# ivannz/cplxmodule

Measured on AMD Instinct MI355X. Metric: Cplx-samples/sec fwd+bwd (CplxLinear-4096 + VD), higher is better.
Workload: dtype bf16; 1 GPU; CplxLinearVD 4096->4096, bf16 activations / fp32 master weights, batch 8192 per GPU, LRT fwd + KL + full bwd (BASELINE configs[1] + VD); global_batch=8192, parallelism=dp1, noise=in-kernel Philox4x32-7, launch=hipGraph replay, warmup_detail=5 eager steps (capture prerequisites) + 5 untimed replays

## Files before the change

cplxmodule_amd/_lib.py:

```python
import ctypes
import os
import threading
from ctypes import c_double, c_float, c_int, c_int64, c_uint64, c_void_p

import torch

_HERE = os.path.dirname(os.path.abspath(__file__))
LIB_PATH = os.environ.get("CPLXAMD_LIB") or os.path.join(_HERE, "libcplxamd.so")
ABI_VERSION = 25

F32, BF16, F16, F64 = 0, 1, 2, 3
KL_KINDS = {"real_vd": 0, "real_ard": 1, "cplx_vd": 2, "cplx_ard": 3, "cplx_vd_approx": 4,
            "cplx_vd_scalefree": 5, "cplx_vd_bogus": 6, "real_l0": 7, "real_l1": 8}

_P, _I, _L, _U, _F, _D = c_void_p, c_int, c_int64, c_uint64, c_float, c_double

SIGNATURES = {
    "cplxamd_abi_version": [],
    "cplxamd_vd_kl_ws_bytes": [],
    "cplxamd_vd_kl_fwd": [_P, _P, _P, _I, _P, _P, _P, _L, _P],
    "cplxamd_vd_kl_bwd": [_P, _P, _P, _I, _P, _P, _P, _P, _P, _L, _P],
    "cplxamd_vd_kl_fwd_bwd": [_P, _P, _P, _I, _F, _P, _P, _P, _P, _P, _L, _P],
    "cplxamd_vd_log_alpha": [_P, _P, _P, _P, _L, _P],
    "cplxamd_vd_log_alpha_bwd": [_P, _P, _P, _P, _P, _L, _P],
# ... 62 lines not shown
    "cplxamd_conv2d_cl2": [_P, _P, _P, _P, _P, _P, _P, _L] + [_I] * 11 + [_P, _L, _P],
    "cplxamd_chansum2": [_P, _P, _P, _P, _L, _I, _L, _I, _P, _P],
    "cplxamd_conv2d_cl2_lrt_dx": [_P] * 8 + [_L] + [_I] * 6 + [_P, _L, _P],
    "cplxamd_conv2d_cl2_mom_chunks": [_L] + [_I] * 10,
    "cplxamd_conv2d_cl2_mom": [_P, _P, _P, _P, _P, _P, _P, _L] + [_I] * 10 + [_P, _L, _P, _L, _P],
    "cplxamd_conv2d_cl_wgrad_ws_bytes": [_L, _I, _I, _I, _I],
    "cplxamd_conv2d_cl_wgrad": [_P, _P, _P, _P, _P, _P, _P, _L] + [_I] * 10 + [_P, _L, _P],
    "cplxamd_cgemm3m_ws_bytes": [_I, _I, _I],
    "cplxamd_abs2": [_P, _P, _P, _L, _I, _I, _P],
    "cplxamd_modulus": [_P, _P, _P, _L, _P],
    "cplxamd_exp": [_P, _P, _L, _I, _P],
    "cplxamd_cast": [_P, _P, _L, _I, _I, _P],
    "cplxamd_split3": [_P, _P, _L, _P, _L, _L, _L, _I, _I, _I, _P],
    "cplxamd_absmax_ws_bytes": [],
    "cplxamd_absmax_scale": [_P, _P, _L, _L, _I, _I, _P, _P, _P],
    "cplxamd_split2h": [_P, _P, _L, _P, _L, _L, _L, _I, _I, _I, _P, _P],
    "cplxamd_cgemm_sc_fl": [_P, _P, _L, _L, _P, _P, _L, _L, _P, _P, _P, _P, _P, _L, _I, _I, _I, _I, _I, _I, _P, _P, _P, _P, _L,
                            _I, _P],
    "cplxamd_rgemm_sc_fl": [_P, _L, _L, _P, _L, _L, _P, _P, _I, _P, _L, _I, _I, _I, _I, _I, _P, _P, _P, _P, _L, _I, _P],
    "cplxamd_transpose": [_P, _L, _P, _L, _I, _I, _I, _P],
    "cplxamd_colsum_ws_bytes": [_I],
    "cplxamd_colsum": [_P, _L, _P, _I, _I, _I, _P, _P],
    "cplxamd_colsum2": [_P, _P, _L, _P, _P, _I, _I, _I, _P, _P],
    "cplxamd_lrt_dx_accum": [_P, _P, _P, _P, _P, _L, _I, _I, _P],
    "cplxamd_conv2d_fwd": [_P, _P, _P, _P, _P, _P, _P, _P, _P, _I, _P],
    "cplxamd_conv2d_dgrad": [_P, _P, _P, _P, _P, _P, _P, _I, _P],
    "cplxamd_conv2d_wgrad_splits": [_P],
    "cplxamd_conv2d_wgrad_ws_bytes": [_P, _I],
    "cplxamd_conv2d_wgrad": [_P, _P, _P, _P, _P, _P, _P, _P, _I, _P, _L, _P],
    "cplxamd_conv2d_wgrad_bias": [_P, _P, _P, _P, _P, _P, _P, _P, _P, _P, _I, _P, _L, _P],
    "cplxamd_conv2d_out_shape": [_P, _P, _P],
    "cplxamd_conv2d_ktab_size": [_P, _I],
    "cplxamd_conv2d_ktab_fill": [_P, _I, _P],
    "cplxamd_conv2d_bf16_fwd": [_P, _P, _P, _P, _P, _P, _P, _P, _P, _P, _P],
    "cplxamd_conv2d_bf16_dgrad": [_P, _P, _P, _P, _P, _P, _P, _P, _P],
    "cplxamd_conv2d_bf16_wgrad_ws_bytes": [_P, _I],
    "cplxamd_conv2d_bf16_wgrad": [_P, _P, _P, _P, _P, _P, _P, _P, _P, _P, _L, _P],
    "cplxamd_chansum": [_P, _P, _L, _I, _L, _I, _P, _P],
    "cplxamd_bn_ws_bytes": [_I],
    "cplxamd_bn_fwd": [_P, _P, _P, _P, _L, _I, _L, _P, _P, _P, _P, _P, _I, _I, _F, _F, _P, _L, _P],
    "cplxamd_bn_fwd_ex": [_P, _P, _P, _P, _L, _I, _L, _P, _P, _P, _P, _P, _I, _I, _F, _F, _P, _P, _L, _P],
    "cplxamd_bn_bwd": [_P, _P, _P, _P, _P, _P, _L, _I, _L, _P, _P, _P, _P, _I, _I, _P, _L, _P],
    "cplxamd_bn_bwd_sums": [_P, _P, _P, _P, _P, _P, _L, _I, _L, _P, _P, _P, _P, _I, _I, _P, _P, _L, _P],
    "cplxamd_bn_rows_path": [_L, _I, _L],
    "cplxamd_gemm_set_persistent": [_I],
    "cplxamd_gemm_set_family": [_I],
    "cplxamd_cgemm_fl": [_P, _P, _L, _L, _P, _P, _L, _L, _P, _P, _P, _P, _P, _L, _I, _I, _I, _I, _I,
                         _I, _I, _P, _I, _P, _L, _I, _P],
    "cplxamd_rgemm_fl": [_P, _L, _L, _P, _L, _L, _P, _P, _I, _P, _L, _I, _I, _I, _I, _I, _I, _P, _P, _L, _I, _P],
    "cplxamd_cgemm_lrt_dx_fl": [_P, _P, _L, _L, _P, _P, _L, _L, _P, _P, _P, _L, _P, _P, _L, _I, _I, _I, _I, _I, _P],
    "cplxamd_rgemm_lrt_dx_fl": [_P, _L, _L, _P, _L, _L, _P, _P, _L, _P, _L, _I, _I, _I, _I, _I, _P],
    "cplxamd_gemm_plan": [_I] * 10,
    "cplxamd_conv2d_cl_fl": [_P, _P, _P, _P, _P, _P, _P, _L] + [_I] * 11 + [_P, _L, _I, _P],
    "cplxamd_conv2d_cl2_fl": [_P, _P, _P, _P, _P, _P, _P, _L] + [_I] * 11 + [_P, _L, _I, _P],
    "cplxamd_conv2d_cl2_lrt_dx_fl": [_P] * 8 + [_L] + [_I] * 6 + [_P, _L, _I, _P],
    "cplxamd_conv2d_cl2_mom_chunks_fl": [_L] + [_I] * 11,
    "cplxamd_conv2d_cl2_mom_fl": [_P, _P, _P, _P, _P, _P, _P, _L] + [_I] * 10 + [_P, _L, _P, _L, _I, _P],
    "cplxamd_conv2d_cl_wgrad_fl": [_P, _P, _P, _P, _P, _P, _P, _L] + [_I] * 10 + [_P, _L, _I, _P],
    "cplxamd_bn_bwd_sums_amax": [_P, _P, _P, _P, _P, _P, _L, _I, _L, _P, _P, _P, _P, _I, _I, _P, _P, _P, _L, _P],
    "cplxamd_absmax_scale_partials": [_P, _I, _P, _P],
    "cplxamd_bn_bwd_coef": [_P, _P, _P, _P, _L, _I, _L, _P, _P, _P, _P, _I, _I, _P, _P, _P, _L, _P],
    "cplxamd_conv2d_cl_wgrad_bn_fl": [_P] * 11 + [_L] + [_I] * 10 + [_P, _L, _I, _P],
    "cplxamd_gemm_f64": [_P, _P, _L, _L, _L, _P, _P, _L, _L, _L, _P, _P, _P, _P, _L, _L, _I, _I, _I, _I, _I, _P],
    "cplxamd_conv2d_f64": [_P, _P, _P, _P, _P, _P, _P, _P, _P, _I, _P],
    "cplxamd_expi_f64": [_P, _P, _L, _P],
    "cplxamd_conv2d_cl2h_fl": [_P, _P, _I, _P, _P, _P, _P, _P, _I, _P, _P, _L] + [_I] * 7 + [_P, _L, _I, _P],
    "cplxamd_conv2d_cl2h_wrap_fl": [_P, _P, _I, _I, _P, _P, _P, _P, _P, _I, _P, _P, _L] + [_I] * 7 + [_P, _L, _I, _P],
    "cplxamd_conv2d_clh_wgrad_ws_bytes": [_L, _I, _I, _I, _I],
    "cplxamd_conv2d_clh_wgrad": [_P, _P, _P, _P, _P, _P, _P, _L] + [_I] * 10 + [_P, _L, _P],
    "cplxamd_conv2d_clh_wgrad_fl": [_P, _P, _P, _P, _P, _P, _P, _L] + [_I] * 10 + [_P, _L, _I, _P],
    "cplxamd_conv2d_clh_wgrad_skip_fl": [_P, _P, _P, _P, _P, _P, _L] + [_I] * 12 + [_P, _L, _I, _P],
    "cplxamd_conv2d_clr_fl": [_P, _P, _P, _P, _L] + [_I] * 11 + [_P, _L, _I, _P],
    "cplxamd_conv2d_clr_wgrad_fl": [_P, _P, _P, _I, _P, _L] + [_I] * 10 + [_P, _L, _I, _P],
    "cplxamd_bn_moments": [_P, _P, _P, _P, _P, _L, _I, _L, _I, _P, _P, _L, _P],
    "cplxamd_bn_fwd_sync": [_P, _P, _P, _P, _L, _I, _L, _P, _P, _P, _P, _P, _I, _F, _F, _P, _P, _P, _L, _P],
    "cplxamd_bn_fwd_partials": [_P, _P, _P, _P, _L, _I, _L, _P, _P, _P, _P, _P, _I, _F, _F, _P, _P, _I, _P, _L, _P],
    "cplxamd_bn_bwd_sync": [_P, _P, _P, _P, _P, _P, _L, _I, _L, _P, _P, _P, _P, _I, _P, _P, _P, _P, _P, _L, _P],
    "cplxamd_cplx_fn_fwd": [_P, _P, _P, _P, _L, _I, _I, _P],
    "cplxamd_cplx_fn_bwd": [_P, _P, _P, _P, _P, _P, _L, _I, _I, _P],
    "cplxamd_welch_plan": [_L, _L, _L, _I, _P, _P],
    "cplxamd_welch_fwd": [_P, _P, _L, _L, _L, _L, _P, _L, _L, _I, _D, _P, _P, _L, _I, _P],
    "cplxamd_welch_bwd": [_P, _P, _L, _L, _L, _L, _P, _L, _L, _I, _D, _P, _P, _P, _L, _L, _P, _L, _I, _P],
    "cplxamd_ceinsum": [_P, _P, _P, _P, _P, _P, _P, _I, _I, _I, _I, _P],
}


class EinsumDesc(ctypes.Structure):
    _fields_ = [("nmodes", ctypes.c_int32 * 4), ("extent", (ctypes.c_int32 * 8) * 4), ("stride_a", (c_int64 * 8) * 4),
                ("stride_b", (c_int64 * 8) * 4), ("stride_c", (c_int64 * 8) * 4)]


CPLX_FN = {"exp": 0, "log": 1, "sin": 2, "cos": 3, "tan": 4, "sinh": 5, "cosh": 6, "tanh": 7}
_RESTYPES = {"cplxamd_absmax_ws_bytes": c_int64, "cplxamd_conv2d_cl2_mom_chunks": c_int64, "cplxamd_conv2d_cl2_mom_chunks_fl": c_int64, "cplxamd_vd_kl_ws_bytes": c_int64, "cplxamd_lrt_reparam_bwd_cols_ws_bytes": c_int64, "cplxamd_l0_gate_bwd_ws_bytes": c_int64, "cplxamd_bn_ws_bytes": c_int64,
             "cplxamd_conv2d_wgrad_ws_bytes": c_int64, "cplxamd_conv2d_bf16_wgrad_ws_bytes": c_int64, "cplxamd_colsum_ws_bytes": c_int64, "cplxamd_gemm_ws_bytes": c_int64,
             "cplxamd_cgemm3m_ws_bytes": c_int64,
             "cplxamd_conv2d_nhwc_wgrad_ws_bytes": c_int64,
             "cplxamd_conv2d_nhwc_wgrad_f32_ws_bytes": c_int64,
             "cplxamd_conv2d_cl_pack_bytes": c_int64, "cplxamd_conv2d_cl_ws_bytes": c_int64,
             "cplxamd_conv2d_cl_wgrad_ws_bytes": c_int64, "cplxamd_conv2d_clh_wgrad_ws_bytes": c_int64,

             "cplxamd_conv2d_clr_pack_bytes": c_int64,
             "cplxamd_conv2d_clr_ws_bytes": c_int64, "cplxamd_conv2d_clr_wgrad_ws_bytes": c_int64}

_lib = None

LAUNCH_DEFAULT, LAUNCH_SHARED, LAUNCH_EXCLUSIVE = 0, 1, 2


def LAUNCH_FAMILY(mask):
    return 0x100 | ((int(mask) & 0xff) << 16)


_policy = {}
_sharing = set()
_policy_lock = threading.Lock()


def _stream_key():
    if not torch.cuda.is_available():
        return (-1, 0)
    idx = torch.cuda.current_device()
    return (idx, _current_stream_handle(idx))


def launch_flags():
    if _policy:
        f = _policy.get(_stream_key())
        if f is not None:
            return f
    return LAUNCH_SHARED if _sharing else LAUNCH_DEFAULT


class launch_policy:

    def __init__(self, flags):
        self.flags = int(flags)

    def __enter__(self):
        self.key = _stream_key()
        with _policy_lock:
            self.prev = _policy.get(self.key)
            _policy[self.key] = self.flags
        return self

    def __exit__(self, *exc):
        with _policy_lock:
            if self.prev is None:
                _policy.pop(self.key, None)
            else:
                _policy[self.key] = self.prev
        return False


def shared_chip_enter(owner):
    with _policy_lock:
        _sharing.add(id(owner))


def shared_chip_leave(owner):
    with _policy_lock:
        _sharing.discard(id(owner))


class CplxAmdError(RuntimeError):
    pass


def load():
    global _lib
    if _lib is not None:
        return _lib
    if not os.path.exists(LIB_PATH):
        raise CplxAmdError(
            f"{LIB_PATH} not found: build it with `python -c 'import __graft_entry__ as g; "
            "g.build()'` (or cplxmodule_amd/csrc/build.sh).  cplxmodule_amd has no CPU or "
            "pure-torch fallback.")
# ... 98 lines not shown
```

cplxmodule_amd/csrc/common.h:

```cpp
#pragma once
#include <hip/hip_runtime.h>
#include <stdint.h>

#include "../../include/cplxamd.h"

#define CPLXAMD_CHECK_LAUNCH()                          \
  do {                                                  \
    hipError_t e__ = hipGetLastError();                 \
    if (e__ != hipSuccess) return (int)e__;             \
  } while (0)

#if defined(CPLXAMD_GEMM_F16) || defined(CPLXAMD_CONV_F16)
typedef _Float16 cplxamd_f16x8 __attribute__((ext_vector_type(8)));
#define CPLXAMD_MFMA16(a, b, c) \
  __builtin_amdgcn_mfma_f32_32x32x16_f16(__builtin_bit_cast(cplxamd_f16x8, a), __builtin_bit_cast(cplxamd_f16x8, b), c, 0, 0, 0)
#else
#define CPLXAMD_MFMA16(a, b, c) __builtin_amdgcn_mfma_f32_32x32x16_bf16(a, b, c, 0, 0, 0)
#endif

namespace cplxamd {

constexpr int kWave = 64;

#ifndef CPLXAMD_PHILOX_ROUNDS
// ... 51 lines not shown
                                             uint32_t lds_off_uniform) {
  const uint64_t a = (uint64_t)(uintptr_t)sbase_uniform;
  const uint64_t lo = (uint32_t)__builtin_amdgcn_readfirstlane((int)(uint32_t)a);
  const uint64_t hi = (uint32_t)__builtin_amdgcn_readfirstlane((int)(uint32_t)(a >> 32));
  const uint64_t sb = (hi << 32) | lo;
  const uint32_t m0v = (uint32_t)__builtin_amdgcn_readfirstlane((int)lds_off_uniform);
  asm volatile("s_mov_b32 m0, %0\n\ts_nop 0\n\tglobal_load_lds_dwordx4 %1, %2"
               :
               : "s"(m0v), "v"(voff), "s"(sb)
               : "memory");
}

struct f4 { float v[4]; };
struct f8 { f4 h[2]; };
__device__ __forceinline__ f4 ld4(const float* p) {
  float4 t = *reinterpret_cast<const float4*>(p);
  return f4{{t.x, t.y, t.z, t.w}};
}
__device__ __forceinline__ void st4(float* p, const f4& a) {
  *reinterpret_cast<float4*>(p) = make_float4(a.v[0], a.v[1], a.v[2], a.v[3]);
}
__device__ __forceinline__ f4 ld4(const bf16_t* p) {
  uint2 t = *reinterpret_cast<const uint2*>(p);
  return f4{{__uint_as_float(t.x << 16), __uint_as_float(t.x & 0xffff0000u),
             __uint_as_float(t.y << 16), __uint_as_float(t.y & 0xffff0000u)}};
}
__device__ __forceinline__ void st4(bf16_t* p, const f4& a) {
  uint2 t;
  t.x = pack_bf16(a.v[0], a.v[1]);
  t.y = pack_bf16(a.v[2], a.v[3]);
  *reinterpret_cast<uint2*>(p) = t;
}
__device__ __forceinline__ f8 ld8(const float* p) { return f8{{ld4(p), ld4(p + 4)}}; }
__device__ __forceinline__ void st8(float* p, const f8& a) { st4(p, a.h[0]); st4(p + 4, a.h[1]); }
__device__ __forceinline__ f8 ld8(const bf16_t* p) {
  const uint4 t = *reinterpret_cast<const uint4*>(p);
  const uint32_t w[4] = {t.x, t.y, t.z, t.w};
  f8 r;
#pragma unroll
  for (int e = 0; e < 4; ++e) {
    r.h[e >> 1].v[(e & 1) * 2] = __uint_as_float(w[e] << 16);
    r.h[e >> 1].v[(e & 1) * 2 + 1] = __uint_as_float(w[e] & 0xffff0000u);
  }
  return r;
}
__device__ __forceinline__ void st8(bf16_t* p, const f8& a) {
  uint32_t w[4];
#pragma unroll
  for (int e = 0; e < 4; ++e)
    w[e] = pack_bf16(a.h[e >> 1].v[(e & 1) * 2], a.h[e >> 1].v[(e & 1) * 2 + 1]);
  *reinterpret_cast<uint4*>(p) = uint4{w[0], w[1], w[2], w[3]};
}

__device__ __forceinline__ float rn_sqrt(float x) { return sqrtf(x); }

__device__ __forceinline__ float exact_logf(float x) {
  double d = (double)x;
  asm volatile("" : "+v"(d));
  return (float)log(d);
}

__device__ __forceinline__ double wave_sum(double v) {
#pragma unroll
  for (int o = 32; o > 0; o >>= 1) v += __shfl_xor(v, o, 64);
  return v;
}
__device__ __forceinline__ float wave_sum(float v) {
#pragma unroll
  for (int o = 32; o > 0; o >>= 1) v += __shfl_xor(v, o, 64);
  return v;
}

template <typename T, int NT>
__device__ __forceinline__ T block_sum(T v, T* smem) {
  v = wave_sum(v);
  const int lane = threadIdx.x & 63, wid = threadIdx.x >> 6;
  if (lane == 0) smem[wid] = v;
  __syncthreads();
  T r = T(0);
  if (threadIdx.x < NT / 64) r = smem[threadIdx.x];
  if (wid == 0) r = wave_sum(r);
  __syncthreads();
  return r;
}

__device__ __forceinline__ uint64_t uniform64(uint64_t v) {
  const uint32_t lo = (uint32_t)__builtin_amdgcn_readfirstlane((int)(uint32_t)v);
  const uint32_t hi = (uint32_t)__builtin_amdgcn_readfirstlane((int)(uint32_t)(v >> 32));
  return ((uint64_t)hi << 32) | lo;
}

struct u32x4 { uint32_t v[4]; };

__device__ __forceinline__ u32x4 philox4x32(uint64_t ctr_lo, uint64_t ctr_hi, uint64_t key) {
  uint32_t c0 = (uint32_t)ctr_lo, c1 = (uint32_t)(ctr_lo >> 32);
  uint32_t c2 = (uint32_t)ctr_hi, c3 = (uint32_t)(ctr_hi >> 32);
  uint32_t k0 = (uint32_t)key, k1 = (uint32_t)(key >> 32);
#pragma unroll
  for (int r = 0; r < kPhiloxRounds; ++r) {
    const uint64_t p0 = (uint64_t)0xD2511F53u * c0, p1 = (uint64_t)0xCD9E8D57u * c2;
    const uint32_t lo0 = (uint32_t)p0, hi0 = (uint32_t)(p0 >> 32);
    const uint32_t lo1 = (uint32_t)p1, hi1 = (uint32_t)(p1 >> 32);
    c0 = __builtin_amdgcn_bitop3_b32(hi1, c1, k0, 0x96);
    c1 = lo1;
    c2 = __builtin_amdgcn_bitop3_b32(hi0, c3, k1, 0x96);
    c3 = lo0;
    k0 += 0x9E3779B9u;
    k1 += 0xBB67AE85u;
  }
  return u32x4{{c0, c1, c2, c3}};
}

__device__ __forceinline__ float u01(uint32_t x) {
  return fmaf((float)(x >> 8), 5.9604644775390625e-08f, 2.98023223876953125e-08f);
}

inline int stream_grid(int64_t work_items, int block) {
  int64_t g = (work_items + block - 1) / block;
  if (g < 1) g = 1;
  if (g > 2048) g = 2048;
  return (int)g;
}

}
```

cplxmodule_amd/csrc/gemm_bf16_w4.hip:

```cpp
#include <stdlib.h>

#include <type_traits>

#include "gemm.h"

namespace cplxamd {
namespace w4 {

typedef __bf16 bf16x8 __attribute__((ext_vector_type(8)));
typedef short s16x4 __attribute__((ext_vector_type(4)));
typedef short s16x8 __attribute__((ext_vector_type(8)));
typedef float f32x16 __attribute__((ext_vector_type(16)));
typedef uint32_t u32x4 __attribute__((ext_vector_type(4)));

#ifndef W4_LDP
#define W4_LDP 0
#endif
#ifndef W4_WAIT1
#define W4_WAIT1 0
#endif
#ifndef W4_LDQ
#define W4_LDQ 0
#endif

// ... 450 lines not shown
        using NR = std::false_type;
        tile(I0{}, I0{}, t, NR{});
        tile(I1{}, I1{}, t + 1, NR{});
        tile(I2{}, I0{}, t + 2, NR{});
        tile(I0{}, I1{}, t + 3, NR{});
        tile(I1{}, I0{}, t + 4, NR{});
        tile(I2{}, I1{}, t + 5, NR{});
      }
    }
    for (; t + 6 <= nt; t += 6) {
      tile(I0{}, I0{}, t, RD{});
      tile(I1{}, I1{}, t + 1, RD{});
      tile(I2{}, I0{}, t + 2, RD{});
      tile(I0{}, I1{}, t + 3, RD{});
      tile(I1{}, I0{}, t + 4, RD{});
      tile(I2{}, I1{}, t + 5, RD{});
    }
    if (t < nt) {
      tile(I0{}, I0{}, t, RD{});
      tile(I1{}, I1{}, t + 1, RD{});
      t += 2;
      if (t < nt) {
        tile(I2{}, I0{}, t, RD{});
        tile(I0{}, I1{}, t + 1, RD{});
        if constexpr (PERSIST) rotate(I1{});
      } else {
        if constexpr (PERSIST) rotate(I2{});
      }
    }
  }

#ifdef CPLXAMD_GEMM_F16
  if constexpr (!PERSIST) {
    if (g.scale_a) {
      const float alpha = gemm_alpha(g);
#pragma unroll
      for (int i = 0; i < IB; ++i)
#pragma unroll
        for (int j = 0; j < JB; ++j) {
          acc_r[i][j] *= alpha;
          if (CPLX) acc_i[i][j] *= alpha;
        }
    }
  }
#endif

  void* out_r = g.c_r;
  void* out_i = g.c_i;
  if (g.splits > 1) {
    const int64_t slab = (int64_t)g.M * g.ldc;
    float* base = reinterpret_cast<float*>(g.ws) + (int64_t)split * NPL * slab;
    out_r = base; out_i = base + slab;
  }
  const float beta = gemm_beta(g);
  asm volatile("s_waitcnt lgkmcnt(0)" ::: "memory");
  if constexpr (!PERSIST) __builtin_amdgcn_s_barrier();
  auto tile_rsrc = [&](const void* plane, int64_t ld, int esize) __attribute__((always_inline)) {
    const char* base = (const char*)plane + ((int64_t)m0 * ld + n0) * esize;
    return __builtin_amdgcn_make_buffer_rsrc((void*)base, 0, 0x7ffffffe, 0x00020000);
  };
  auto ldb128 = [](__amdgpu_buffer_rsrc_t r, uint32_t vo, uint32_t so) __attribute__((always_inline)) -> u32x4 {
    return __builtin_amdgcn_raw_buffer_load_b128(r, vo, so, 0);
  };
  auto stb128 = [](u32x4 v, __amdgpu_buffer_rsrc_t r, uint32_t vo, uint32_t so) __attribute__((always_inline)) {
    __builtin_amdgcn_raw_buffer_store_b128(v, r, vo, so, 0);
  };
  if constexpr (sizeof(TOUT) == 2) {
    auto epi16 = [&](auto FUSE) __attribute__((always_inline)) {
      constexpr bool fuse = decltype(FUSE)::value;
      constexpr int PITCH = 144;
      const int tid_e = PERSIST ? (int)opaque((uint32_t)tid) : tid;
      const int lane = tid_e & 63, wid = tid_e >> 6;
      const int wm = (wid / C::WN) * (32 * IB), wn = (wid % C::WN) * (32 * JB);
      const int l31 = lane & 31, lk = lane >> 5;
      const uint32_t vo_c = (uint32_t)((((int64_t)(wm + (lane >> 3)) * g.ldc + wn + (lane & 7) * 8)) * 2);
      char* reg = smem + (PERSIST ? (CPLX ? sl[2] : (uint32_t)C::SMEM) : 0u) + wid * (64 * PITCH);
      const uint32_t vo_f = fuse ? (uint32_t)((((int64_t)(wm + (lane >> 3)) * g.fld + wn + (lane & 7) * 8)) * 2) : 0u;
      const uint32_t p8c = (uint32_t)__builtin_amdgcn_readfirstlane((int)(uint32_t)(8 * g.ldc * 2));
      const uint32_t p8f = (uint32_t)__builtin_amdgcn_readfirstlane((int)(uint32_t)(8 * g.fld * 2));
      const __amdgpu_buffer_rsrc_t rga = tile_rsrc(fuse ? g.fga : g.c_r, fuse ? g.fld : g.ldc, 2);
      const __amdgpu_buffer_rsrc_t rout0 = tile_rsrc(out_r, g.ldc, 2), rout1 = tile_rsrc(CPLX ? out_i : out_r, g.ldc, 2);
      const __amdgpu_buffer_rsrc_t rx0 = tile_rsrc(fuse ? g.fx_r : g.c_r, fuse ? g.fld : g.ldc, 2);
      const __amdgpu_buffer_rsrc_t rx1 = tile_rsrc(fuse ? (CPLX ? g.fx_i : g.fx_r) : g.c_r, fuse ? g.fld : g.ldc, 2);
      constexpr int NR = NPL * (JB / 2) * (IB / 2);
      u32x4 gv[2][fuse ? 8 : 1], xv[2][fuse ? 8 : 1];
      auto load_ops = [&](int r) __attribute__((always_inline)) {
        const int pl = r / ((JB / 2) * (IB / 2)), jh = (r / (IB / 2)) % (JB / 2), ih = r % (IB / 2);
#pragma unroll
        for (int pass = 0; pass < 8; ++pass) {
          const uint32_t so = (uint32_t)(ih * 8 + pass) * p8f + (uint32_t)(jh * 128);
          gv[r & 1][pass] = ldb128(rga, vo_f, so);
          xv[r & 1][pass] = ldb128(pl ? rx1 : rx0, vo_f, so);
        }
      };
      if constexpr (fuse) load_ops(0);
      if constexpr (PERSIST) W4_VMCNT(0);
#pragma unroll
      for (int r = 0; r < NR; ++r) {
        const int pl = r / ((JB / 2) * (IB / 2)), jh = (r / (IB / 2)) % (JB / 2), ih = r % (IB / 2);
        const __amdgpu_buffer_rsrc_t rout = pl ? rout1 : rout0;
        if constexpr (fuse && !W4_EPI_PIPE) { if (r > 0) load_ops(r); }
#pragma unroll
        for (int ii = 0; ii < 2; ++ii)
#pragma unroll
          for (int jj = 0; jj < 2; ++jj)
#pragma unroll
            for (int q = 0; q < 4; ++q) {
              const int cl = jj * 32 + 8 * q + 4 * lk;
              f4 v;
#pragma unroll
              for (int e = 0; e < 4; ++e) {
                const float a = pl ? acc_i[CPLX ? ih * 2 + ii : 0][jh * 2 + jj][4 * q + e] : acc_r[ih * 2 + ii][jh * 2 + jj][4 * q + e];
                v.v[e] = a;
              }
              st4(reinterpret_cast<bf16_t*>(reg + (ii * 32 + l31) * PITCH + cl * 2), v);
              if constexpr (PERSIST) W4_SB();
            }
        asm volatile("s_waitcnt lgkmcnt(0)" ::: "memory");
        if constexpr (fuse && W4_EPI_PIPE) {
          if (r + 1 < NR) { W4_SB(); load_ops(r + 1); W4_SB(); }
        }
#pragma unroll
        for (int pass = 0; pass < 8; ++pass) {
          const int rl = pass * 8 + (lane >> 3), c8 = (lane & 7) * 8;
          const u32x4 v = *reinterpret_cast<const u32x4*>(reg + rl * PITCH + c8 * 2);
          const uint32_t so = (uint32_t)(ih * 8 + pass) * p8c + (uint32_t)(jh * 128);
          if constexpr (fuse) {
            u32x4 ow;
#pragma unroll
            for (int e = 0; e < 4; ++e) {
              const float d0 = __uint_as_float(v[e] << 16), d1 = __uint_as_float(v[e] & 0xffff0000u);
              const float x0 = __uint_as_float(xv[r & 1][pass][e] << 16), x1 = __uint_as_float(xv[r & 1][pass][e] & 0xffff0000u);
              const float g0 = __uint_as_float(gv[r & 1][pass][e] << 16), g1 = __uint_as_float(gv[r & 1][pass][e] & 0xffff0000u);
              ow[e] = pack_bf16(fmaf(2.0f * x0, g0, d0), fmaf(2.0f * x1, g1, d1));
            }
            stb128(ow, rout, vo_c, so);
          } else {
            stb128(v, rout, vo_c, so);
          }
        }
        asm volatile("s_waitcnt lgkmcnt(0)" ::: "memory");
        if constexpr (PERSIST) W4_VMCNT(16);
        W4_SB();
      }
    };
    if constexpr (PERSIST) epi16(std::false_type{});
    else { if (g.fga) epi16(std::true_type{}); else epi16(std::false_type{}); }
  } else {
    auto epi32 = [&](auto HM, auto HACC) __attribute__((always_inline)) {
      constexpr bool hm = decltype(HM)::value, hacc = decltype(HACC)::value;
      constexpr int PITCH = 272;
      char* reg = smem + wid * (32 * PITCH);
      const uint32_t vo = (uint32_t)((((int64_t)(wm + (lane >> 4)) * g.ldc + wn + (lane & 15) * 4)) * 4);
      const uint32_t p4 = (uint32_t)__builtin_amdgcn_readfirstlane((int)(uint32_t)(4 * g.ldc * 4));
      const __amdgpu_buffer_rsrc_t rm = tile_rsrc(hm ? (const void*)g.emul : g.c_r, g.ldc, 4);
      const __amdgpu_buffer_rsrc_t rout0 = tile_rsrc(out_r, g.ldc, 4), rout1 = tile_rsrc(CPLX ? out_i : out_r, g.ldc, 4);
      constexpr int NR = NPL * (JB / 2) * IB;
      u32x4 mv[2][hm ? 8 : 1], pv[2][hacc ? 8 : 1];
      auto load_ops = [&](int r) __attribute__((always_inline)) {
        const int pl = r / ((JB / 2) * IB), jh = (r / IB) % (JB / 2), i = r % IB;
#pragma unroll
        for (int pass = 0; pass < 8; ++pass) {
          const uint32_t so = (uint32_t)(i * 8 + pass) * p4 + (uint32_t)(jh * 256);
          if constexpr (hm) mv[r & 1][pass] = ldb128(rm, vo, so);
          if constexpr (hacc) pv[r & 1][pass] = ldb128(pl ? rout1 : rout0, vo, so);
        }
      };
      if constexpr (hm || hacc) load_ops(0);
#pragma unroll
      for (int r = 0; r < NR; ++r) {
        const int pl = r / ((JB / 2) * IB), jh = (r / IB) % (JB / 2), i = r % IB;
        const __amdgpu_buffer_rsrc_t rout = pl ? rout1 : rout0;
        if constexpr ((hm || hacc) && !W4_EPI_PIPE) { if (r > 0) load_ops(r); }
#pragma unroll
        for (int jj = 0; jj < 2; ++jj)
#pragma unroll
          for (int q = 0; q < 4; ++q) {
            const int cl = jj * 32 + 8 * q + 4 * lk;
            f4 v;
#pragma unroll
            for (int e = 0; e < 4; ++e)
              v.v[e] = pl ? acc_i[CPLX ? i : 0][jh * 2 + jj][4 * q + e] : acc_r[i][jh * 2 + jj][4 * q + e];
            st4(reinterpret_cast<float*>(reg + l31 * PITCH + cl * 4), v);
          }
        asm volatile("s_waitcnt lgkmcnt(0)" ::: "memory");
        if constexpr ((hm || hacc) && W4_EPI_PIPE) {
          if (r + 1 < NR) { W4_SB(); load_ops(r + 1); W4_SB(); }
        }
#pragma unroll
        for (int pass = 0; pass < 8; ++pass) {
          const int rl = pass * 4 + (lane >> 4), c4 = (lane & 15) * 4;
          f4 v = ld4(reinterpret_cast<const float*>(reg + rl * PITCH + c4 * 4));
          const uint32_t so = (uint32_t)(i * 8 + pass) * p4 + (uint32_t)(jh * 256);
          if constexpr (hm) {
#pragma unroll
            for (int e = 0; e < 4; ++e) {
              v.v[e] *= gemm_emul(g, __uint_as_float(mv[r & 1][pass][e]));
              asm volatile("" : "+v"(v.v[e]));
            }
          }
          if constexpr (hacc) {
#pragma unroll
            for (int e = 0; e < 4; ++e) v.v[e] += beta * __uint_as_float(pv[r & 1][pass][e]);
          }
          const u32x4 w = {__float_as_uint(v.v[0]), __float_as_uint(v.v[1]), __float_as_uint(v.v[2]), __float_as_uint(v.v[3])};
          stb128(w, rout, vo, so);
        }
        asm volatile("s_waitcnt lgkmcnt(0)" ::: "memory");
        W4_SB();
      }
    };
    if (g.emul) { if (g.accumulate) epi32(std::true_type{}, std::true_type{}); else epi32(std::true_type{}, std::false_type{}); }
    else { if (g.accumulate) epi32(std::false_type{}, std::true_type{}); else epi32(std::false_type{}, std::false_type{}); }
  }
  if constexpr (!PERSIST) {
    break;
// ... 144 lines not shown
```

cplxmodule_amd/csrc/kl.hip:

```cpp
#include "common.h"

#pragma clang fp contract(off)

namespace cplxamd {

constexpr int kKlThreads = 256;
constexpr int kKlMaxBlocks = 2048;
#ifndef KL_UNROLL
#define KL_UNROLL 1
#endif
#ifndef KL_NT
#define KL_NT 3
#endif

constexpr float kEulerGamma = 0.57721566490153286f;
constexpr float kK1 = 0.63576f, kK2 = 1.87320f, kK3 = 1.48695f;

template <bool CPLX, bool EXACT = true>
__device__ __forceinline__ float weight_abs(float wr, float wi) {
  if (CPLX) return EXACT ? rn_sqrt(fmaf(wi, wi, wr * wr)) : __builtin_amdgcn_sqrtf(fmaf(wi, wi, wr * wr));
  return fabsf(wr);
}

template <bool CPLX, bool EXACT>
// ... 96 lines not shown
template <int KIND>
__device__ __forceinline__ float one_param_value(float p, float& slope) {
  if (KIND == CPLXAMD_KL_REAL_L0) {
    const float s = sigmoid_f(kL0Shift - p);
    slope = -(s * (1.0f - s));
    return s;
  }
  slope = p > 0.0f ? 1.0f : (p < 0.0f ? -1.0f : 0.0f);
  return fabsf(p);
}

template <bool CPLX>
__device__ __forceinline__ void weight_grad(float fp, float wr, float wi, float theta,
                                            float& gwr, float& gwi) {
  if (theta > 0.0f) {
    if (CPLX) {
      const float c = 2.0f * fp * __builtin_amdgcn_rcpf(theta * (theta + 1e-12f));
      gwr = c * wr;
      gwi = c * wi;
    } else {
      gwr = (wr < 0.0f ? -2.0f : 2.0f) * fp / (theta + 1e-12f);
      gwi = 0.0f;
    }
  } else {
    gwr = 0.0f;
    gwi = 0.0f;
  }
}

typedef float f2 __attribute__((ext_vector_type(2)));
__device__ __forceinline__ f2 fma2(f2 a, f2 b, f2 c) { return __builtin_elementwise_fma(a, b, c); }
__device__ __forceinline__ f2 sp2(float v) { return f2{v, v}; }
__device__ __forceinline__ f2 sel2(bool c0, bool c1, f2 a, f2 b) { return f2{c0 ? a.x : b.x, c1 ? a.y : b.y}; }

__device__ __forceinline__ float exp_neg(float ls) {
  const float yh = -ls * 1.44269504089f;
  const float yl = fmaf(-ls, 1.44269504089f, -yh);
  const float e = __builtin_amdgcn_exp2f(yh);
  return fmaf(e, yl * 0.69314718056f, e);
}

__device__ __forceinline__ void cplx_vd_pair(f2 x, f2& val, f2& slope) {
  f2 s = sp2(3.0619244e-7f);
  s = fma2(s, x, sp2(-3.1001984e-6f));
  s = fma2(s, x, sp2(2.8344671e-5f));
  s = fma2(s, x, sp2(-2.3148148e-4f));
  s = fma2(s, x, sp2(1.6666667e-3f));
  s = fma2(s, x, sp2(-1.0416667e-2f));
  s = fma2(s, x, sp2(5.5555556e-2f));
  s = fma2(s, x, sp2(-0.25f));
  s = fma2(s, x, sp2(1.0f));
  const f2 small = s * x;
  const f2 num = fma2(fma2(fma2(x + sp2(8.5733287401f), x, sp2(18.0590169730f)), x, sp2(8.6347608925f)), x, sp2(0.2677737343f));
  const f2 den = fma2(fma2(fma2(x + sp2(9.5733223454f), x, sp2(25.6329561486f)), x, sp2(21.0996530827f)), x, sp2(3.9584969228f));
  const f2 xd = x * den;
  const f2 nx = x * sp2(-1.44269504089f);
  const f2 e = f2{__builtin_amdgcn_exp2f(nx.x), __builtin_amdgcn_exp2f(nx.y)};
  const f2 rc = f2{__builtin_amdgcn_rcpf(xd.x), __builtin_amdgcn_rcpf(xd.y)};
  const f2 lg = f2{__builtin_amdgcn_logf(x.x), __builtin_amdgcn_logf(x.y)} * sp2(0.69314718056f);
  f2 e1 = e * num * rc;
  e1 = sel2(x.x < 104.0f, x.y < 104.0f, e1, sp2(0.0f));
  const f2 large = sp2(kEulerGamma) + lg + e1;
  val = sel2(x.x <= 1.0f, x.y <= 1.0f, small, large);
  const f2 ss = fma2(fma2(x, sp2(1.6666667e-1f), sp2(-0.5f)), x, sp2(1.0f)) * x;
  slope = sel2(x.x < 0.015625f, x.y < 0.015625f, ss, sp2(1.0f) - e);
}

struct KlArgs {
  const float* wr;
  const float* wi;
  const float* ls2;
  const float* g_elem;
  const float* g_scalar;
  float gscale;
  float* out_elem;
  double* partial;
  float* g_ls2;
  float* g_wr;
  float* g_wi;
  int64_t n;
  bf16_t* wr_b = nullptr;
  bf16_t* wi_b = nullptr;
  bf16_t* s_b = nullptr;
};

__device__ __forceinline__ void st4g(float* p, const f4& v) {
#if KL_NT & 1
  typedef float f4v __attribute__((ext_vector_type(4)));
  __builtin_nontemporal_store(f4v{v.v[0], v.v[1], v.v[2], v.v[3]}, reinterpret_cast<f4v*>(p));
#else
  st4(p, v);
#endif
}
__device__ __forceinline__ f4 ld4g(const float* p) {
#if KL_NT & 2
  typedef float f4v __attribute__((ext_vector_type(4)));
  const f4v t = __builtin_nontemporal_load(reinterpret_cast<const f4v*>(p));
  return f4{{t.x, t.y, t.z, t.w}};
#else
  return ld4(p);
#endif
}

template <int KIND, bool VALUE, bool GRAD>
__global__ __launch_bounds__(kKlThreads) void kl_kernel(KlArgs a) {
  constexpr bool CPLX = KIND >= CPLXAMD_KL_CPLX_VD && KIND <= CPLXAMD_KL_CPLX_VD_BOGUS;
  constexpr float kLs = kl_ls2_term<KIND>();
  __shared__ double red[kKlThreads / 64];
  const int64_t n4 = a.n >> 2;
  const int64_t stride = (int64_t)gridDim.x * kKlThreads;
  float gs = a.gscale;
  if (GRAD && a.g_scalar) gs *= *a.g_scalar;
  double acc = 0.0;

  auto body = [&](int64_t i, const f4& wr, const f4& ls, const f4& wi, const f4& ge) __attribute__((always_inline)) {
    f4 val, d_ls, d_wr, d_wi;
    float part = 0.0f;
    bool done = false;
    if constexpr (KIND == CPLXAMD_KL_CPLX_VD) {
      float q[4];
      bool tiny = false;
#pragma unroll
      for (int j = 0; j < 4; ++j) {
        q[j] = fmaf(wi.v[j], wi.v[j], wr.v[j] * wr.v[j]);
        tiny |= !(q[j] >= 1e-8f);
      }
#pragma unroll
      for (int h = 0; h < 2; ++h) {
        const f2 x = f2{q[2 * h] * exp_neg(ls.v[2 * h]), q[2 * h + 1] * exp_neg(ls.v[2 * h + 1])};
        f2 v, sl;
        cplx_vd_pair(x, v, sl);
        if (VALUE) { val.v[2 * h] = v.x; val.v[2 * h + 1] = v.y; }
        if (GRAD) {
          const f2 fp = sl * f2{ge.v[2 * h], ge.v[2 * h + 1]} * sp2(gs);
          const f2 c = (fp + fp) * f2{__builtin_amdgcn_rcpf(q[2 * h]), __builtin_amdgcn_rcpf(q[2 * h + 1])};
          d_ls.v[2 * h] = -fp.x; d_ls.v[2 * h + 1] = -fp.y;
          d_wr.v[2 * h] = c.x * wr.v[2 * h]; d_wr.v[2 * h + 1] = c.y * wr.v[2 * h + 1];
          d_wi.v[2 * h] = c.x * wi.v[2 * h]; d_wi.v[2 * h + 1] = c.y * wi.v[2 * h + 1];
        }
      }
      done = !tiny;
      if (VALUE && done) part = (val.v[0] + val.v[1]) + (val.v[2] + val.v[3]);
    }
    if constexpr (kl_one_param<KIND>()) {
#pragma unroll
      for (int j = 0; j < 4; ++j) {
        float sl;
        const float v = one_param_value<KIND>(KIND == CPLXAMD_KL_REAL_L0 ? ls.v[j] : wr.v[j], sl);
        if (VALUE) { val.v[j] = v; part += v; }
        if (GRAD) {
          const float g = sl * ge.v[j] * gs;
          d_ls.v[j] = KIND == CPLXAMD_KL_REAL_L0 ? g : 0.0f;
          d_wr.v[j] = KIND == CPLXAMD_KL_REAL_L1 ? g : 0.0f;
          d_wi.v[j] = 0.0f;
        }
      }
      done = true;
    }
    if (!done) {
      part = 0.0f;
#pragma unroll
      for (int j = 0; j < 4; ++j) {
        float theta;
        const float t = -log_alpha_of<CPLX, false>(ls.v[j], wr.v[j], wi.v[j], theta);
        if (VALUE) {
          val.v[j] = kl_value<KIND>(t) + kLs * ls.v[j];
// ... 4 lines not shown
          d_ls.v[j] = kLs * ge.v[j] * gs - fp;
          weight_grad<CPLX>(fp, wr.v[j], wi.v[j], theta, d_wr.v[j], d_wi.v[j]);
        }
      }
    }
    if (VALUE) {
      acc += (double)part;
      if (a.out_elem) st4(a.out_elem + 4 * i, val);
    }
    if (GRAD) {
      if (a.g_ls2) st4g(a.g_ls2 + 4 * i, d_ls);
      if (a.g_wr) st4g(a.g_wr + 4 * i, d_wr);
      if (CPLX && a.g_wi) st4g(a.g_wi + 4 * i, d_wi);
    }
    if (a.wr_b) st4(a.wr_b + 4 * i, wr);
    if (CPLX && a.wi_b) st4(a.wi_b + 4 * i, wi);
    if (a.s_b) {
      f4 e;
#pragma unroll
      for (int j = 0; j < 4; ++j) e.v[j] = expf(ls.v[j]);
      st4(a.s_b + 4 * i, e);
    }
  };
  for (int64_t i0 = (int64_t)blockIdx.x * kKlThreads + threadIdx.x; i0 < n4; i0 += KL_UNROLL * stride) {
    f4 wr[KL_UNROLL], ls[KL_UNROLL], wi[KL_UNROLL], ge[KL_UNROLL];
#pragma unroll
    for (int u = 0; u < KL_UNROLL; ++u) {
      const int64_t i = i0 + u * stride;
      wi[u] = f4{{0.f, 0.f, 0.f, 0.f}};
      ge[u] = f4{{1.f, 1.f, 1.f, 1.f}};
      if (i < n4) {
        wr[u] = ld4g(a.wr + 4 * i);
        ls[u] = ld4g(a.ls2 + 4 * i);
        if (CPLX) wi[u] = ld4g(a.wi + 4 * i);
        if (GRAD && a.g_elem) ge[u] = ld4(a.g_elem + 4 * i);
      }
    }
#pragma unroll
    for (int u = 0; u < KL_UNROLL; ++u) {
      const int64_t i = i0 + u * stride;
      if (i < n4) body(i, wr[u], ls[u], wi[u], ge[u]);
    }
  }
  if (blockIdx.x == 0) {
    const int64_t i = (n4 << 2) + threadIdx.x;
    if (i < a.n) {
      const float wr = a.wr[i], ls = a.ls2[i];
      const float wi = CPLX ? a.wi[i] : 0.0f;
      if constexpr (kl_one_param<KIND>()) {
        float sl;
        const float v = one_param_value<KIND>(KIND == CPLXAMD_KL_REAL_L0 ? ls : wr, sl);
        if (VALUE) {
          acc += (double)v;
          if (a.out_elem) a.out_elem[i] = v;
        }
        if (GRAD) {
          const float g = sl * (a.g_elem ? a.g_elem[i] : 1.0f) * gs;
          if (a.g_ls2) a.g_ls2[i] = KIND == CPLXAMD_KL_REAL_L0 ? g : 0.0f;
          if (a.g_wr) a.g_wr[i] = KIND == CPLXAMD_KL_REAL_L1 ? g : 0.0f;
        }
      } else {
      float theta;
      const float t = -log_alpha_of<CPLX, false>(ls, wr, wi, theta);
      if (VALUE) {
        const float v = kl_value<KIND>(t) + kLs * ls;
        acc += (double)v;
        if (a.out_elem) a.out_elem[i] = v;
      }
      if (GRAD) {
        const float ge = a.g_elem ? a.g_elem[i] : 1.0f;
        const float fp = kl_slope<KIND>(t) * ge * gs;
        float gwr, gwi;
        weight_grad<CPLX>(fp, wr, wi, theta, gwr, gwi);
        if (a.g_ls2) a.g_ls2[i] = kLs * ge * gs - fp;
        if (a.g_wr) a.g_wr[i] = gwr;
        if (CPLX && a.g_wi) a.g_wi[i] = gwi;
      }
      }
    }
  }
  if (VALUE && a.partial) {
    const double s = block_sum<double, kKlThreads>(acc, red);
    if (threadIdx.x == 0) a.partial[blockIdx.x] = s;
  }
}

__global__ __launch_bounds__(kKlThreads) void kl_final_kernel(const double* partial, int m,
                                                              float* out) {
  __shared__ double red[kKlThreads / 64];
  double acc = 0.0;
  for (int i = threadIdx.x; i < m; i += kKlThreads) acc += partial[i];
  const double s = block_sum<double, kKlThreads>(acc, red);
  if (threadIdx.x == 0) *out = (float)s;
}

template <bool VALUE, bool GRAD>
static int launch_kl(int kind, const KlArgs& a, int grid, hipStream_t st) {
  switch (kind) {
    case CPLXAMD_KL_REAL_VD:
      kl_kernel<CPLXAMD_KL_REAL_VD, VALUE, GRAD><<<grid, kKlThreads, 0, st>>>(a);
      break;
    case CPLXAMD_KL_REAL_ARD:
      kl_kernel<CPLXAMD_KL_REAL_ARD, VALUE, GRAD><<<grid, kKlThreads, 0, st>>>(a);
      break;
    case CPLXAMD_KL_CPLX_VD:
      kl_kernel<CPLXAMD_KL_CPLX_VD, VALUE, GRAD><<<grid, kKlThreads, 0, st>>>(a);
      break;
    case CPLXAMD_KL_CPLX_ARD:
      kl_kernel<CPLXAMD_KL_CPLX_ARD, VALUE, GRAD><<<grid, kKlThreads, 0, st>>>(a);
      break;
    case CPLXAMD_KL_CPLX_VD_APPROX:
      kl_kernel<CPLXAMD_KL_CPLX_VD_APPROX, VALUE, GRAD><<<grid, kKlThreads, 0, st>>>(a);
      break;
    case CPLXAMD_KL_CPLX_VD_SCALEFREE:
      kl_kernel<CPLXAMD_KL_CPLX_VD_SCALEFREE, VALUE, GRAD><<<grid, kKlThreads, 0, st>>>(a);
      break;
    case CPLXAMD_KL_CPLX_VD_BOGUS:
      kl_kernel<CPLXAMD_KL_CPLX_VD_BOGUS, VALUE, GRAD><<<grid, kKlThreads, 0, st>>>(a);
      break;
    case CPLXAMD_KL_REAL_L0:
      kl_kernel<CPLXAMD_KL_REAL_L0, VALUE, GRAD><<<grid, kKlThreads, 0, st>>>(a);
      break;
    case CPLXAMD_KL_REAL_L1:
      kl_kernel<CPLXAMD_KL_REAL_L1, VALUE, GRAD><<<grid, kKlThreads, 0, st>>>(a);
      break;
    default:
      return CPLXAMD_EINVAL;
  }
  CPLXAMD_CHECK_LAUNCH();
  return 0;
}

__global__ __launch_bounds__(kKlThreads) void prep_kernel(const float* wr, const float* wi, const float* ls2,
                                                          bf16_t* wr_b, bf16_t* wi_b, bf16_t* s_b, int64_t n) {
  const int64_t n4 = n >> 2, stride = (int64_t)gridDim.x * kKlThreads;
  for (int64_t i = (int64_t)blockIdx.x * kKlThreads + threadIdx.x; i < n4; i += stride) {
    if (wr_b) st4(wr_b + 4 * i, ld4(wr + 4 * i));
    if (wi_b) st4(wi_b + 4 * i, ld4(wi + 4 * i));
    if (s_b) {
      f4 e = ld4(ls2 + 4 * i);
#pragma unroll
      for (int j = 0; j < 4; ++j) e.v[j] = expf(e.v[j]);
      st4(s_b + 4 * i, e);
    }
  }
}

static bool kl_args_ok(const float* wr, const float* wi, const float* ls2, int kind, int64_t n) {
  if (!wr || !ls2 || n < 0 || kind < 0 || kind > CPLXAMD_KL_REAL_L1) return false;
  const bool cplx = kind >= CPLXAMD_KL_CPLX_VD && kind <= CPLXAMD_KL_CPLX_VD_BOGUS;
  return cplx ? wi != nullptr : true;
}

template <bool CPLX, bool MASK>
__global__ __launch_bounds__(kKlThreads) void log_alpha_kernel(const float* wr, const float* wi,
                                                               const float* ls2, float thr,
                                                               float* out, double* partial,
                                                               int64_t n) {
  __shared__ double red[kKlThreads / 64];
  const int64_t n4 = n >> 2;
  const int64_t stride = (int64_t)gridDim.x * kKlThreads;
  double cnt = 0.0;
  for (int64_t i = (int64_t)blockIdx.x * kKlThreads + threadIdx.x; i < n4; i += stride) {
    const f4 a = ld4(wr + 4 * i), l = ld4(ls2 + 4 * i);
    f4 b = {{0.f, 0.f, 0.f, 0.f}};
    if (CPLX) b = ld4(wi + 4 * i);
    f4 o;
    float c = 0.0f;
#pragma unroll
    for (int j = 0; j < 4; ++j) {
      float theta;
      const float la = log_alpha_of<CPLX, true>(l.v[j], a.v[j], b.v[j], theta);
      o.v[j] = MASK ? (la <= thr ? 1.0f : 0.0f) : la;
      c += MASK ? o.v[j] : 0.0f;
    }
    st4(out + 4 * i, o);
    cnt += (double)c;
  }
  if (blockIdx.x == 0) {
    const int64_t i = (n4 << 2) + threadIdx.x;
    if (i < n) {
      float theta;
      const float la = log_alpha_of<CPLX, true>(ls2[i], wr[i], CPLX ? wi[i] : 0.0f, theta);
      const float o = MASK ? (la <= thr ? 1.0f : 0.0f) : la;
      out[i] = o;
      if (MASK) cnt += (double)o;
    }
  }
  if (MASK && partial) {
    const double s = block_sum<double, kKlThreads>(cnt, red);
    if (threadIdx.x == 0) partial[blockIdx.x] = s;
  }
}

template <bool CPLX>
__global__ __launch_bounds__(kKlThreads) void log_alpha_bwd_kernel(const float* g, const float* wr,
                                                                   const float* wi, float* g_wr, float* g_wi,
                                                                   int64_t n) {
  const int64_t stride = (int64_t)gridDim.x * kKlThreads;
  for (int64_t i = (int64_t)blockIdx.x * kKlThreads + threadIdx.x; i < n; i += stride) {
    const float a = wr[i], b = CPLX ? wi[i] : 0.0f;
    const float theta = weight_abs<CPLX, true>(a, b);
    float ga, gb;
    weight_grad<CPLX>(-g[i], a, b, theta, ga, gb);
    g_wr[i] = ga;
    if (CPLX) g_wi[i] = gb;
  }
}

__global__ __launch_bounds__(kKlThreads) void count_final_kernel(const double* partial, int m,
                                                                 int64_t* out) {
  __shared__ double red[kKlThreads / 64];
  double acc = 0.0;
  for (int i = threadIdx.x; i < m; i += kKlThreads) acc += partial[i];
  const double s = block_sum<double, kKlThreads>(acc, red);
  if (threadIdx.x == 0) *out = (int64_t)(s + 0.5);
}

__device__ __forceinline__ float expi_f(float xf) {
  const double x = (double)xf;
  if (xf == 0.0f) return -INFINITY;
  if (xf < 0.0f) {
    const double y = -x;
    if (y <= 1.0) {
      double s = 0.0, term = 1.0;
      for (int k = 1; k <= 20; ++k) {
        term *= -y / k;
        s += term / k;
      }
      return (float)(0.57721566490153286 + log(y) + s);
    }
    if (y > 745.0) return -0.0f;
    double b = y + 1.0, c = 1e300, d = 1.0 / b, h = d;
    for (int i = 1; i <= 60; ++i) {
      const double an = -(double)i * i;
      b += 2.0;
      d = 1.0 / (an * d + b);
      c = b + an / c;
      const double del = c * d;
      h *= del;
      if (fabs(del - 1.0) < 1e-15) break;
    }
    return (float)(-h * exp(-y));
  }
  if (x <= 40.0) {
    double s = 0.0, term = 1.0;
    for (int k = 1; k <= 200; ++k) {
      term *= x / k;
      const double add = term / k;
      s += add;
      if (add < s * 1e-17) break;
    }
    return (float)(0.57721566490153286 + log(x) + s);
  }
  double s = 1.0, term = 1.0;
  for (int k = 1; k <= 40; ++k) {
    const double nt = term * k / x;
    if (nt > term) break;
    term = nt;
    s += term;
  }
  return (float)(exp(x) / x * s);
}

__global__ __launch_bounds__(kKlThreads) void expi_fwd_kernel(const float* x, float* y, int64_t n) {
  const int64_t stride = (int64_t)gridDim.x * kKlThreads;
  for (int64_t i = (int64_t)blockIdx.x * kKlThreads + threadIdx.x; i < n; i += stride)
    y[i] = expi_f(x[i]);
}
__global__ __launch_bounds__(kKlThreads) void expi_bwd_kernel(const float* g, const float* x,
                                                              float* gx, int64_t n) {
  const int64_t stride = (int64_t)gridDim.x * kKlThreads;
  for (int64_t i = (int64_t)blockIdx.x * kKlThreads + threadIdx.x; i < n; i += stride)
    gx[i] = g[i] * expf(x[i]) / x[i];
}

}

using namespace cplxamd;

extern "C" {

int cplxamd_abi_version(void) { return CPLXAMD_ABI_VERSION; }

int64_t cplxamd_vd_kl_ws_bytes(void) { return (int64_t)kKlMaxBlocks * sizeof(double); }

int cplxamd_vd_kl_fwd(const float* wr, const float* wi, const float* log_sigma2, int kind,
                      float* out_elem, float* out_sum, void* ws, int64_t n, void* stream) {
  if (!kl_args_ok(wr, wi, log_sigma2, kind, n) || (out_sum && !ws)) return CPLXAMD_EINVAL;
  hipStream_t st = (hipStream_t)stream;
  const int grid = stream_grid(n >> 2, kKlThreads);
  KlArgs a{wr, wi, log_sigma2, nullptr, nullptr, 1.0f, out_elem,
           out_sum ? (double*)ws : nullptr, nullptr, nullptr, nullptr, n};
  int rc = launch_kl<true, false>(kind, a, grid, st);
  if (rc) return rc;
  if (out_sum) {
    kl_final_kernel<<<1, kKlThreads, 0, st>>>((const double*)ws, grid, out_sum);
    CPLXAMD_CHECK_LAUNCH();
  }
  return 0;
}

int cplxamd_vd_kl_bwd(const float* wr, const float* wi, const float* log_sigma2, int kind,
                      const float* g_elem, const float* g_scalar, float* g_log_sigma2,
                      float* g_wr, float* g_wi, int64_t n, void* stream) {
  if (!kl_args_ok(wr, wi, log_sigma2, kind, n)) return CPLXAMD_EINVAL;
  const int grid = stream_grid(n >> 2, kKlThreads);
  KlArgs a{wr, wi, log_sigma2, g_elem, g_scalar, 1.0f, nullptr, nullptr,
           g_log_sigma2, g_wr, g_wi, n};
  return launch_kl<false, true>(kind, a, grid, (hipStream_t)stream);
}

int cplxamd_vd_kl_fwd_bwd(const float* wr, const float* wi, const float* log_sigma2, int kind,
                          float gscale, float* out_sum, float* g_log_sigma2, float* g_wr,
                          float* g_wi, void* ws, int64_t n, void* stream) {
  if (!kl_args_ok(wr, wi, log_sigma2, kind, n) || !out_sum || !ws) return CPLXAMD_EINVAL;
  hipStream_t st = (hipStream_t)stream;
  const int grid = stream_grid(n >> 2, kKlThreads);
  KlArgs a{wr, wi, log_sigma2, nullptr, nullptr, gscale, nullptr, (double*)ws,
           g_log_sigma2, g_wr, g_wi, n};
  int rc = launch_kl<true, true>(kind, a, grid, st);
  if (rc) return rc;
  kl_final_kernel<<<1, kKlThreads, 0, st>>>((const double*)ws, grid, out_sum);
  CPLXAMD_CHECK_LAUNCH();
  return 0;
}

int cplxamd_vd_prep_kl(const float* wr, const float* wi, const float* log_sigma2, int kind, int with_kl,
                       void* wr_bf16, void* wi_bf16, void* s_bf16, float* out_sum, float* g_log_sigma2,
                       float* g_wr, float* g_wi, void* ws, int64_t n, void* stream) {
  if (n < 0 || (n & 3)) return CPLXAMD_ESHAPE;
  if ((wr_bf16 && !wr) || (wi_bf16 && !wi) || (s_bf16 && !log_sigma2)) return CPLXAMD_EINVAL;
  hipStream_t st = (hipStream_t)stream;
  const int grid = stream_grid(n >> 2, kKlThreads);
  if (!with_kl) {
    prep_kernel<<<grid, kKlThreads, 0, st>>>(wr, wi, log_sigma2, (bf16_t*)wr_bf16, (bf16_t*)wi_bf16,
                                             (bf16_t*)s_bf16, n);
    CPLXAMD_CHECK_LAUNCH();
    return 0;
  }
  if (!kl_args_ok(wr, wi, log_sigma2, kind, n) || !out_sum || !ws) return CPLXAMD_EINVAL;
  KlArgs a{wr, wi, log_sigma2, nullptr, nullptr, 1.0f, nullptr, (double*)ws,
           g_log_sigma2, g_wr, g_wi, n};
  a.wr_b = (bf16_t*)wr_bf16; a.wi_b = (bf16_t*)wi_bf16; a.s_b = (bf16_t*)s_bf16;
  int rc = launch_kl<true, true>(kind, a, grid, st);
  if (rc) return rc;
  kl_final_kernel<<<1, kKlThreads, 0, st>>>((const double*)ws, grid, out_sum);
  CPLXAMD_CHECK_LAUNCH();
  return 0;
}

int cplxamd_vd_log_alpha(const float* wr, const float* wi, const float* log_sigma2, float* out,
                         int64_t n, void* stream) {
  if (!wr || !log_sigma2 || !out || n < 0) return CPLXAMD_EINVAL;
  hipStream_t st = (hipStream_t)stream;
  const int grid = stream_grid(n >> 2, kKlThreads);
  if (wi)
    log_alpha_kernel<true, false><<<grid, kKlThreads, 0, st>>>(wr, wi, log_sigma2, 0.f, out,
                                                               nullptr, n);
  else
    log_alpha_kernel<false, false><<<grid, kKlThreads, 0, st>>>(wr, wi, log_sigma2, 0.f, out,
                                                                nullptr, n);
  CPLXAMD_CHECK_LAUNCH();
  return 0;
}

int cplxamd_vd_log_alpha_bwd(const float* g, const float* wr, const float* wi, float* g_wr, float* g_wi,
                             int64_t n, void* stream) {
  if (!g || !wr || !g_wr || n < 0 || ((wi == nullptr) != (g_wi == nullptr))) return CPLXAMD_EINVAL;
  hipStream_t st = (hipStream_t)stream;
  const int grid = stream_grid(n, kKlThreads);
  if (wi) log_alpha_bwd_kernel<true><<<grid, kKlThreads, 0, st>>>(g, wr, wi, g_wr, g_wi, n);
  else log_alpha_bwd_kernel<false><<<grid, kKlThreads, 0, st>>>(g, wr, wi, g_wr, g_wi, n);
  CPLXAMD_CHECK_LAUNCH();
  return 0;
}

int cplxamd_vd_mask(const float* wr, const float* wi, const float* log_sigma2, float threshold,
                    float* mask, int64_t* count, void* ws, int64_t n, void* stream) {
  if (!wr || !log_sigma2 || !mask || n < 0 || (count && !ws)) return CPLXAMD_EINVAL;
  hipStream_t st = (hipStream_t)stream;
  const int grid = stream_grid(n >> 2, kKlThreads);
  double* partial = count ? (double*)ws : nullptr;
  if (wi)
    log_alpha_kernel<true, true><<<grid, kKlThreads, 0, st>>>(wr, wi, log_sigma2, threshold,
                                                              mask, partial, n);
  else
    log_alpha_kernel<false, true><<<grid, kKlThreads, 0, st>>>(wr, wi, log_sigma2, threshold,
                                                               mask, partial, n);
  CPLXAMD_CHECK_LAUNCH();
  if (count) {
    count_final_kernel<<<1, kKlThreads, 0, st>>>(partial, grid, count);
    CPLXAMD_CHECK_LAUNCH();
  }
  return 0;
}

int cplxamd_expi_fwd(const float* x, float* y, int64_t n, void* stream) {
  if (!x || !y || n < 0) return CPLXAMD_EINVAL;
  expi_fwd_kernel<<<stream_grid(n, kKlThreads), kKlThreads, 0, (hipStream_t)stream>>>(x, y, n);
  CPLXAMD_CHECK_LAUNCH();
  return 0;
}

int cplxamd_expi_bwd(const float* g, const float* x, float* gx, int64_t n, void* stream) {
  if (!g || !x || !gx || n < 0) return CPLXAMD_EINVAL;
  expi_bwd_kernel<<<stream_grid(n, kKlThreads), kKlThreads, 0, (hipStream_t)stream>>>(g, x, gx, n);
  CPLXAMD_CHECK_LAUNCH();
  return 0;
}

}
```

cplxmodule_amd/csrc/reparam.hip:

```cpp
#include "common.h"

#pragma clang fp contract(off)

namespace cplxamd {

constexpr int kRpThreads = 256;

__device__ __forceinline__ void box_muller(uint32_t a, uint32_t b, float scale, float& z0,
                                           float& z1) {
  const float r = __builtin_amdgcn_sqrtf((-1.3862943611198906f * scale * scale) * __builtin_amdgcn_logf(u01(a)));
  const float ang = u01(b);
  z0 = r * __builtin_amdgcn_cosf(ang);
  z1 = r * __builtin_amdgcn_sinf(ang);
}

__device__ __forceinline__ f4 philox_normals(uint64_t group, uint64_t seed, uint64_t offset,
                                             float scale) {
  const u32x4 x = philox4x32(group, offset, seed);
  f4 z;
  box_muller(x.v[0], x.v[1], scale, z.v[0], z.v[1]);
  box_muller(x.v[2], x.v[3], scale, z.v[2], z.v[3]);
  return z;
}

constexpr float kRsqrt2 = 0.70710678118654752f;

template <bool CPLX>
__device__ __forceinline__ void noise_vec(int64_t i4, uint64_t seed, uint64_t offset, f4& er,
                                          f4& ei) {
  if (CPLX) {
    const f4 a = philox_normals(2 * (uint64_t)i4, seed, offset, kRsqrt2);
    const f4 b = philox_normals(2 * (uint64_t)i4 + 1, seed, offset, kRsqrt2);
    er = f4{{a.v[0], a.v[2], b.v[0], b.v[2]}};
    ei = f4{{a.v[1], a.v[3], b.v[1], b.v[3]}};
  } else {
    er = philox_normals((uint64_t)i4, seed, offset, 1.0f);
  }
}

template <bool CPLX>
__device__ __forceinline__ void noise_one(int64_t e, uint64_t seed, uint64_t offset, float& er,
                                          float& ei) {
  if (CPLX) {
    const f4 a = philox_normals((uint64_t)e >> 1, seed, offset, kRsqrt2);
    er = (e & 1) ? a.v[2] : a.v[0];
    ei = (e & 1) ? a.v[3] : a.v[1];
  } else {
    const f4 a = philox_normals((uint64_t)e >> 2, seed, offset, 1.0f);
    er = a.v[e & 3];
    ei = 0.0f;
  }
}

__device__ __forceinline__ float lrt_std(float s2) { return rn_sqrt(fmaxf(s2, 1e-8f)); }

template <typename T> __device__ __forceinline__ float lrt_std_t(float s2) {
  if (sizeof(T) == 2) return __builtin_amdgcn_sqrtf(fmaxf(s2, 1e-8f));
  return lrt_std(s2);
}

template <typename T, typename TS, bool CPLX, bool PHILOX>
__global__ __launch_bounds__(kRpThreads) void reparam_fwd_kernel(
    const T* mu_r, const T* mu_i, const TS* s2, const T* eps_r, const T* eps_i, uint64_t seed,
    uint64_t offset, const uint64_t* state, T* y_r, T* y_i, int64_t n) {
  if (PHILOX && state) { seed = uniform64(state[0]); offset = uniform64(state[1]); }
  const int64_t n8 = n >> 3;
  const int64_t stride = (int64_t)gridDim.x * kRpThreads;
  for (int64_t i = (int64_t)blockIdx.x * kRpThreads + threadIdx.x; i < n8; i += stride) {
    const f8 s = ld8(s2 + 8 * i);
    const f8 mr = ld8(mu_r + 8 * i);
    f8 mi, er, ei, yr, yi;
    if (CPLX) mi = ld8(mu_i + 8 * i);
    if (!PHILOX) {
      er = ld8(eps_r + 8 * i);
      if (CPLX) ei = ld8(eps_i + 8 * i);
    }
#pragma unroll
    for (int h = 0; h < 2; ++h) {
      if (PHILOX) noise_vec<CPLX>(2 * i + h, seed, offset, er.h[h], ei.h[h]);
#pragma unroll
      for (int j = 0; j < 4; ++j) {
        const float sd = lrt_std_t<T>(s.h[h].v[j]);
        yr.h[h].v[j] = mr.h[h].v[j] + er.h[h].v[j] * sd;
        if (CPLX) yi.h[h].v[j] = mi.h[h].v[j] + ei.h[h].v[j] * sd;
      }
    }
    st8(y_r + 8 * i, yr);
    if (CPLX) st8(y_i + 8 * i, yi);
  }
  if (blockIdx.x == 0) {
    const int64_t e = (n8 << 3) + threadIdx.x;
    if (e < n) {
      float er, ei = 0.0f;
      if (PHILOX) {
        noise_one<CPLX>(e, seed, offset, er, ei);
      } else {
        er = io<T>::ld(eps_r + e);
        if (CPLX) ei = io<T>::ld(eps_i + e);
      }
      const float sd = lrt_std_t<T>(io<TS>::ld(s2 + e));
      io<T>::st(y_r + e, io<T>::ld(mu_r + e) + er * sd);
      if (CPLX) io<T>::st(y_i + e, io<T>::ld(mu_i + e) + ei * sd);
    }
  }
}

__device__ __forceinline__ float lrt_gs2(float gs, float s2) {
  return s2 >= 1e-8f ? (gs * 0.5f) / lrt_std(s2) : 0.0f;
}
template <typename T> __device__ __forceinline__ float lrt_gs2_t(float gs, float s2) {
  if (sizeof(T) == 2) return s2 >= 1e-8f ? (gs * 0.5f) * __builtin_amdgcn_rsqf(s2) : 0.0f;
  return lrt_gs2(gs, s2);
}

template <typename T, typename TG, typename TS, bool CPLX, bool PHILOX>
__global__ __launch_bounds__(kRpThreads) void reparam_bwd_kernel(
    const T* g_r, const T* g_i, const TS* s2, const T* eps_r, const T* eps_i, uint64_t seed,
    uint64_t offset, const uint64_t* state, TG* g_s2, int64_t n) {
  if (PHILOX && state) { seed = uniform64(state[0]); offset = uniform64(state[1]); }
  const int64_t n8 = n >> 3;
  const int64_t stride = (int64_t)gridDim.x * kRpThreads;
  for (int64_t i = (int64_t)blockIdx.x * kRpThreads + threadIdx.x; i < n8; i += stride) {
    const f8 s = ld8(s2 + 8 * i);
    const f8 gr = ld8(g_r + 8 * i);
    f8 gi, er, ei, o;
    if (CPLX) gi = ld8(g_i + 8 * i);
    if (!PHILOX) {
      er = ld8(eps_r + 8 * i);
      if (CPLX) ei = ld8(eps_i + 8 * i);
    }
#pragma unroll
    for (int h = 0; h < 2; ++h) {
      if (PHILOX) noise_vec<CPLX>(2 * i + h, seed, offset, er.h[h], ei.h[h]);
#pragma unroll
      for (int j = 0; j < 4; ++j) {
        float gs = gr.h[h].v[j] * er.h[h].v[j];
        if (CPLX) gs = gs + gi.h[h].v[j] * ei.h[h].v[j];
        o.h[h].v[j] = lrt_gs2_t<T>(gs, s.h[h].v[j]);
      }
    }
    st8(g_s2 + 8 * i, o);
  }
  if (blockIdx.x == 0) {
    const int64_t e = (n8 << 3) + threadIdx.x;
    if (e < n) {
      float er, ei = 0.0f;
      if (PHILOX) {
        noise_one<CPLX>(e, seed, offset, er, ei);
      } else {
        er = io<T>::ld(eps_r + e);
        if (CPLX) ei = io<T>::ld(eps_i + e);
      }
      float gs = io<T>::ld(g_r + e) * er;
      if (CPLX) gs = gs + io<T>::ld(g_i + e) * ei;
      io<TG>::st(g_s2 + e, lrt_gs2_t<T>(gs, io<TS>::ld(s2 + e)));
    }
  }
}

template <typename T, typename TG, typename TS, bool CPLX, bool PHILOX>
__global__ __launch_bounds__(kRpThreads) void reparam_bwd_cols_kernel(
    const T* g_r, const T* g_i, const TS* s2, const T* eps_r, const T* eps_i, uint64_t seed,
    uint64_t offset, const uint64_t* state, TG* g_s2, int64_t rows, int cols, int64_t rows_per_chunk,
    float* partial) {
  __shared__ float red[kRpThreads * 16];
  if (PHILOX && state) { seed = uniform64(state[0]); offset = uniform64(state[1]); }
  const int CG = cols >> 3;
  const int TX = CG < kRpThreads ? CG : kRpThreads, TY = kRpThreads / TX;
  const int tx = (int)threadIdx.x % TX, ty = (int)threadIdx.x / TX;
  const int col = (int)blockIdx.x * (kRpThreads * 8) + tx * 8;
  const int64_t r0 = (int64_t)blockIdx.y * rows_per_chunk;
  const int64_t r1 = r0 + rows_per_chunk < rows ? r0 + rows_per_chunk : rows;
  constexpr int NP = CPLX ? 2 : 1;
  float acc[NP][8];
#pragma unroll
  for (int p = 0; p < NP; ++p)
#pragma unroll
    for (int c = 0; c < 8; ++c) acc[p][c] = 0.0f;
  for (int64_t r = r0 + ty; r < r1; r += TY) {
    const int64_t i = (r * cols + col) >> 3;
    const f8 s = ld8(s2 + 8 * i);
    const f8 gr = ld8(g_r + 8 * i);
    f8 gi, er, ei, o;
    if (CPLX) gi = ld8(g_i + 8 * i);
    if (!PHILOX) {
      er = ld8(eps_r + 8 * i);
      if (CPLX) ei = ld8(eps_i + 8 * i);
    }
#pragma unroll
    for (int h = 0; h < 2; ++h) {
      if (PHILOX) noise_vec<CPLX>(2 * i + h, seed, offset, er.h[h], ei.h[h]);
#pragma unroll
      for (int j = 0; j < 4; ++j) {
        float gs = gr.h[h].v[j] * er.h[h].v[j];
        if (CPLX) gs = gs + gi.h[h].v[j] * ei.h[h].v[j];
        o.h[h].v[j] = lrt_gs2_t<T>(gs, s.h[h].v[j]);
        acc[0][4 * h + j] += gr.h[h].v[j];
        if (CPLX) acc[NP - 1][4 * h + j] += gi.h[h].v[j];
      }
    }
    st8(g_s2 + 8 * i, o);
  }
  float* dst = partial + (int64_t)blockIdx.y * NP * cols;
  if (TY == 1) {
#pragma unroll
    for (int p = 0; p < NP; ++p) {
      st4(dst + (int64_t)p * cols + col, f4{{acc[p][0], acc[p][1], acc[p][2], acc[p][3]}});
      st4(dst + (int64_t)p * cols + col + 4, f4{{acc[p][4], acc[p][5], acc[p][6], acc[p][7]}});
    }
    return;
  }
#pragma unroll
  for (int p = 0; p < NP; ++p)
#pragma unroll
    for (int c = 0; c < 8; ++c) red[((ty * NP + p) * TX + tx) * 8 + c] = acc[p][c];
  __syncthreads();
  for (int f = (int)threadIdx.x; f < NP * cols; f += kRpThreads) {
    const int p = f / cols, c = f % cols;
    float t = 0.0f;
    for (int l = 0; l < TY; ++l) t += red[((l * NP + p) * TX) * 8 + c];
    dst[(int64_t)p * cols + c] = t;
  }
}

__global__ __launch_bounds__(1024) void reparam_cols_final(const float* partial, int chunks, int cols, int planes,
                                                           float* out_r, float* out_i) {
  __shared__ float red[64][17];
  const int tx = threadIdx.x & 15, ty = threadIdx.x >> 4;
  const int c = blockIdx.x * 16 + tx, n = planes * cols;
  float acc = 0.f;
  if (c < n)
    for (int j = ty; j < chunks; j += 64) acc += partial[(int64_t)j * n + c];
  red[ty][tx] = acc;
  __syncthreads();
  if (ty == 0 && c < n) {
    float t = 0.f;
#pragma unroll 8
    for (int l = 0; l < 64; ++l) t += red[l][tx];
    if (c < cols) out_r[c] = t;
    else out_i[c - cols] = t;
  }
}

struct ColsPlan { int strips, chunks; int64_t rows_per_chunk; };
static bool cols_plan(int64_t rows, int cols, ColsPlan& p) {
  if (rows <= 0 || cols < 8 || cols % 8) return false;
  const int cg = cols / 8;
  if (cg < kRpThreads ? (kRpThreads % cg != 0) : (cols % (kRpThreads * 8) != 0)) return false;
  if (rows * (int64_t)cols >= ((int64_t)1 << 40)) return false;
  p.strips = cg < kRpThreads ? 1 : cols / (kRpThreads * 8);
  const int ty = cg < kRpThreads ? kRpThreads / cg : 1;
  int64_t chunks = rows / (16 * (int64_t)ty);
  const int64_t cap = 2048 / p.strips > 0 ? 2048 / p.strips : 1;
  if (chunks > cap) chunks = cap;
  if (chunks < 1) chunks = 1;
  int64_t rpc = (rows + chunks - 1) / chunks;
  rpc = (rpc + ty - 1) / ty * ty;
  p.rows_per_chunk = rpc;
  p.chunks = (int)((rows + rpc - 1) / rpc);
  return p.chunks <= 65535;
}

template <typename T, typename TG, typename TS>
static int launch_bwd_cols(const void* g_r, const void* g_i, const void* s2, const void* eps_r,
                           const void* eps_i, uint64_t seed, uint64_t offset, const uint64_t* state,
                           void* g_s2, int64_t rows, int cols, const ColsPlan& p, float* partial, hipStream_t st) {
  const dim3 grid((unsigned)p.strips, (unsigned)p.chunks);
  const bool cplx = g_i != nullptr, philox = eps_r == nullptr;
#define RP_BWDC(C, P)                                                                          \
  reparam_bwd_cols_kernel<T, TG, TS, C, P><<<grid, kRpThreads, 0, st>>>(                       \
      (const T*)g_r, (const T*)g_i, (const TS*)s2, (const T*)eps_r, (const T*)eps_i, seed, offset, \
      state, (TG*)g_s2, rows, cols, p.rows_per_chunk, partial)
  if (cplx && philox) RP_BWDC(true, true);
  else if (cplx) RP_BWDC(true, false);
  else if (philox) RP_BWDC(false, true);
  else RP_BWDC(false, false);
#undef RP_BWDC
  CPLXAMD_CHECK_LAUNCH();
  return 0;
}

template <bool CPLX>
__global__ __launch_bounds__(kRpThreads) void philox_normal_kernel(float* er, float* ei,
                                                                   uint64_t seed, uint64_t offset,
                                                                   int64_t n) {
  const int64_t stride = (int64_t)gridDim.x * kRpThreads;
  for (int64_t e = (int64_t)blockIdx.x * kRpThreads + threadIdx.x; e < n; e += stride) {
    float a, b;
    noise_one<CPLX>(e, seed, offset, a, b);
    er[e] = a;
    if (CPLX) ei[e] = b;
  }
}

template <typename T, typename TS>
static int launch_fwd(const void* mu_r, const void* mu_i, const void* s2, const void* eps_r,
                      const void* eps_i, uint64_t seed, uint64_t offset, const uint64_t* state,
                      void* y_r, void* y_i, int64_t n, hipStream_t st) {
  const int grid = stream_grid(n >> 3, kRpThreads);
  const bool cplx = mu_i != nullptr, philox = eps_r == nullptr;
#define RP_FWD(C, P)                                                                       \
  reparam_fwd_kernel<T, TS, C, P><<<grid, kRpThreads, 0, st>>>(                            \
      (const T*)mu_r, (const T*)mu_i, (const TS*)s2, (const T*)eps_r, (const T*)eps_i, seed, offset,  \
      state, (T*)y_r, (T*)y_i, n)
  if (cplx && philox) RP_FWD(true, true);
  else if (cplx) RP_FWD(true, false);
  else if (philox) RP_FWD(false, true);
  else RP_FWD(false, false);
#undef RP_FWD
  CPLXAMD_CHECK_LAUNCH();
  return 0;
}

template <typename T, typename TG, typename TS>
static int launch_bwd(const void* g_r, const void* g_i, const void* s2, const void* eps_r,
                      const void* eps_i, uint64_t seed, uint64_t offset, const uint64_t* state,
                      void* g_s2, int64_t n, hipStream_t st) {
  const int grid = stream_grid(n >> 3, kRpThreads);
  const bool cplx = g_i != nullptr, philox = eps_r == nullptr;
#define RP_BWD(C, P)                                                                      \
  reparam_bwd_kernel<T, TG, TS, C, P><<<grid, kRpThreads, 0, st>>>(                       \
      (const T*)g_r, (const T*)g_i, (const TS*)s2, (const T*)eps_r, (const T*)eps_i, seed, offset,   \
      state, (TG*)g_s2, n)
  if (cplx && philox) RP_BWD(true, true);
  else if (cplx) RP_BWD(true, false);
  else if (philox) RP_BWD(false, true);
  else RP_BWD(false, false);
#undef RP_BWD
  CPLXAMD_CHECK_LAUNCH();
  return 0;
}

__global__ void philox_advance_kernel(uint64_t* state, uint64_t* used) {
  if (threadIdx.x == 0 && blockIdx.x == 0) {
    used[0] = state[0];
    used[1] = state[1];
    state[1] = state[1] + 1;
  }
}

}

using namespace cplxamd;

static bool al16(const void* p) { return (reinterpret_cast<uintptr_t>(p) & 15) == 0; }

extern "C" {

int cplxamd_lrt_reparam_fwd_ex(const void* mu_r, const void* mu_i, const void* s2,
                               const void* eps_r, const void* eps_i, uint64_t seed,
                               uint64_t offset, const uint64_t* state, void* y_r, void* y_i,
                               int64_t n, int dtype, int s2_dtype, void* stream) {
  if (!mu_r || !s2 || !y_r || n < 0) return CPLXAMD_EINVAL;
  if (!al16(mu_r) || !al16(mu_i) || !al16(s2) || !al16(eps_r) || !al16(eps_i) || !al16(y_r) || !al16(y_i))
    return CPLXAMD_EALIGN;
  if ((mu_i == nullptr) != (y_i == nullptr)) return CPLXAMD_EINVAL;
  if (eps_r && mu_i && !eps_i) return CPLXAMD_EINVAL;
  hipStream_t st = (hipStream_t)stream;
  if (dtype == CPLXAMD_F32 && s2_dtype == CPLXAMD_F32)
    return launch_fwd<float, float>(mu_r, mu_i, s2, eps_r, eps_i, seed, offset, state, y_r, y_i, n, st);
  if (dtype == CPLXAMD_BF16 && s2_dtype == CPLXAMD_F32)
    return launch_fwd<bf16_t, float>(mu_r, mu_i, s2, eps_r, eps_i, seed, offset, state, y_r, y_i, n, st);
  if (dtype == CPLXAMD_BF16 && s2_dtype == CPLXAMD_BF16)
    return launch_fwd<bf16_t, bf16_t>(mu_r, mu_i, s2, eps_r, eps_i, seed, offset, state, y_r, y_i, n, st);
  return CPLXAMD_EINVAL;
}

int cplxamd_lrt_reparam_fwd(const void* mu_r, const void* mu_i, const float* s2,
                            const void* eps_r, const void* eps_i, uint64_t seed,
                            uint64_t offset, const uint64_t* state, void* y_r, void* y_i,
                            int64_t n, int dtype, void* stream) {
  return cplxamd_lrt_reparam_fwd_ex(mu_r, mu_i, s2, eps_r, eps_i, seed, offset, state, y_r, y_i, n, dtype,
                                    CPLXAMD_F32, stream);
}

int cplxamd_lrt_reparam_bwd_ex(const void* g_r, const void* g_i, const void* s2,
                               const void* eps_r, const void* eps_i, uint64_t seed,
                               uint64_t offset, const uint64_t* state, void* g_s2, int64_t n,
                               int dtype, int gs2_dtype, int s2_dtype, void* stream) {
  if (!g_r || !s2 || !g_s2 || n < 0) return CPLXAMD_EINVAL;
  if (eps_r && g_i && !eps_i) return CPLXAMD_EINVAL;
  if (!al16(g_r) || !al16(g_i) || !al16(s2) || !al16(eps_r) || !al16(eps_i) || !al16(g_s2))
    return CPLXAMD_EALIGN;
  hipStream_t st = (hipStream_t)stream;
  if (dtype == CPLXAMD_F32 && gs2_dtype == CPLXAMD_F32 && s2_dtype == CPLXAMD_F32)
    return launch_bwd<float, float, float>(g_r, g_i, s2, eps_r, eps_i, seed, offset, state, g_s2, n, st);
  if (dtype == CPLXAMD_BF16 && gs2_dtype == CPLXAMD_F32 && s2_dtype == CPLXAMD_F32)
    return launch_bwd<bf16_t, float, float>(g_r, g_i, s2, eps_r, eps_i, seed, offset, state, g_s2, n, st);
  if (dtype == CPLXAMD_BF16 && gs2_dtype == CPLXAMD_BF16 && s2_dtype == CPLXAMD_F32)
    return launch_bwd<bf16_t, bf16_t, float>(g_r, g_i, s2, eps_r, eps_i, seed, offset, state, g_s2, n, st);
  if (dtype == CPLXAMD_BF16 && gs2_dtype == CPLXAMD_BF16 && s2_dtype == CPLXAMD_BF16)
    return launch_bwd<bf16_t, bf16_t, bf16_t>(g_r, g_i, s2, eps_r, eps_i, seed, offset, state, g_s2, n, st);
  if (dtype == CPLXAMD_BF16 && gs2_dtype == CPLXAMD_F32 && s2_dtype == CPLXAMD_BF16)
    return launch_bwd<bf16_t, float, bf16_t>(g_r, g_i, s2, eps_r, eps_i, seed, offset, state, g_s2, n, st);
  return CPLXAMD_EINVAL;
}

int cplxamd_lrt_reparam_bwd(const void* g_r, const void* g_i, const float* s2,
                            const void* eps_r, const void* eps_i, uint64_t seed,
                            uint64_t offset, const uint64_t* state, void* g_s2, int64_t n,
                            int dtype, int gs2_dtype, void* stream) {
  return cplxamd_lrt_reparam_bwd_ex(g_r, g_i, s2, eps_r, eps_i, seed, offset, state, g_s2, n, dtype, gs2_dtype,
                                    CPLXAMD_F32, stream);
}

int64_t cplxamd_lrt_reparam_bwd_cols_ws_bytes(int64_t rows, int cols) {
  ColsPlan p;
  if (!cols_plan(rows, cols, p)) return 0;
  return (int64_t)p.chunks * 2 * cols * (int64_t)sizeof(float);
}

int cplxamd_lrt_reparam_bwd_cols(const void* g_r, const void* g_i, const void* s2,
                                 const void* eps_r, const void* eps_i, uint64_t seed,
                                 uint64_t offset, const uint64_t* state, void* g_s2, int64_t rows,
                                 int cols, int dtype, int gs2_dtype, int s2_dtype, float* sum_r,
                                 float* sum_i, void* ws, int64_t ws_bytes, void* stream) {
  if (!g_r || !s2 || !g_s2 || !sum_r || !ws || rows < 0) return CPLXAMD_EINVAL;
  if ((g_i == nullptr) != (sum_i == nullptr)) return CPLXAMD_EINVAL;
  if (eps_r && g_i && !eps_i) return CPLXAMD_EINVAL;
  ColsPlan p;
  if (!cols_plan(rows, cols, p)) return CPLXAMD_ESHAPE;
  if (!al16(g_r) || !al16(g_i) || !al16(s2) || !al16(eps_r) || !al16(eps_i) || !al16(g_s2) || !al16(ws))
    return CPLXAMD_EALIGN;
  if (ws_bytes < cplxamd_lrt_reparam_bwd_cols_ws_bytes(rows, cols)) return CPLXAMD_EWS;
  hipStream_t st = (hipStream_t)stream;
  float* partial = (float*)ws;
  int rc = CPLXAMD_EINVAL;
#define RP_GO(T, TG, TS) \
  rc = launch_bwd_cols<T, TG, TS>(g_r, g_i, s2, eps_r, eps_i, seed, offset, state, g_s2, rows, cols, p, partial, st)
  if (dtype == CPLXAMD_F32 && gs2_dtype == CPLXAMD_F32 && s2_dtype == CPLXAMD_F32) RP_GO(float, float, float);
  else if (dtype == CPLXAMD_BF16 && gs2_dtype == CPLXAMD_F32 && s2_dtype == CPLXAMD_F32) RP_GO(bf16_t, float, float);
  else if (dtype == CPLXAMD_BF16 && gs2_dtype == CPLXAMD_BF16 && s2_dtype == CPLXAMD_F32) RP_GO(bf16_t, bf16_t, float);
  else if (dtype == CPLXAMD_BF16 && gs2_dtype == CPLXAMD_BF16 && s2_dtype == CPLXAMD_BF16) RP_GO(bf16_t, bf16_t, bf16_t);
  else if (dtype == CPLXAMD_BF16 && gs2_dtype == CPLXAMD_F32 && s2_dtype == CPLXAMD_BF16) RP_GO(bf16_t, float, bf16_t);
#undef RP_GO
  if (rc) return rc;
  const int planes = g_i ? 2 : 1;
  reparam_cols_final<<<(planes * cols + 15) / 16, 1024, 0, st>>>(partial, p.chunks, cols, planes, sum_r, sum_i);
  CPLXAMD_CHECK_LAUNCH();
  return 0;
}

int cplxamd_philox_advance(uint64_t* state, uint64_t* used, void* stream) {
  if (!state || !used) return CPLXAMD_EINVAL;
  philox_advance_kernel<<<1, 64, 0, (hipStream_t)stream>>>(state, used);
  CPLXAMD_CHECK_LAUNCH();
  return 0;
// ... 17 lines not shown
```

cplxmodule_amd/nn/relevance/complex.py:

```python
import torch

from .base import BaseARD, KLFusion
from .noise import noise
from ..utils.sparsity import SparsityStats
from ..modules.linear import CplxLinear, CplxBilinear
from ..modules.conv import CplxConv1d, CplxConv2d, CplxConv3d
from ... import ops, cplx


def torch_expi(x):
    return ops.ExpiFn.apply(x)


ExpiFunction = ops.ExpiFn


class _CplxGaussianMixin(KLFusion):

    _kl_kind = "cplx_vd"
    __sparsity_ignore__ = ("log_sigma2",)

    def _init_variational(self):
        self.log_sigma2 = torch.nn.Parameter(torch.empty(*self.weight.shape))
        self.reset_variational_parameters()

    def reset_variational_parameters(self):
        self.log_sigma2.data.fill_(-10.0)

    @property
    def log_alpha(self):
        w = self.weight
        return ops.LogAlphaFn.apply(self.log_sigma2, w.real, w.imag)

    @property
    def penalty(self):
        w = self.weight
        return ops.PenaltyFn.apply(self._kl_kind, self.log_sigma2, w.real, w.imag)

    def _penalty_reduced(self, reduction):
        w = self.weight
        total = self._kl_get((w.real, w.imag, self.log_sigma2))
        if total is None:
            total = ops.PenaltySumFn.apply(self._kl_kind, self.log_sigma2, w.real, w.imag)
        return total / self.log_sigma2.numel() if reduction == "mean" else total

    def relevance(self, *, threshold, **kwargs):
        w = self.weight
        with torch.no_grad():
            return ops.relevance_mask(w.real, w.imag, self.log_sigma2, threshold)

    def sparsity(self, *, threshold, **kwargs):
        w = self.weight
        with torch.no_grad():
            _, kept = ops.relevance_mask(w.real, w.imag, self.log_sigma2, threshold, count=True)
        n_dropped = float(w.real.numel()) - float(kept.item())
        return [(id(w.real), n_dropped), (id(w.imag), n_dropped)]

    def _draw_noise(self, shape, like):
        if noise.mode == "torch":
            e = cplx.randn(*shape, dtype=like.dtype, device=like.device)
            return e.real, e.imag, 0, 0
        if noise.mode == "tape":
            e = noise.pop_tape(shape, like, True)
            return e[0], e[1], 0, 0
        seed, offset = noise.next(like.device)
        return None, None, seed, offset


class CplxLinearGaussian(_CplxGaussianMixin, CplxLinear):
    def __init__(self, in_features, out_features, bias=True):
        super().__init__(in_features, out_features, bias=bias)
        self._init_variational()

    def forward(self, input, eps=None):
        if not self.training:
            return super().forward(input)
        w, b = self.weight, self.bias
        if eps is not None:
            er, ei, seed, offset = eps.real, eps.imag, 0, 0
        else:
            er, ei, seed, offset = self._draw_noise((*input.shape[:-1], self.out_features), input)
        br, bi = (None, None) if b is None else (b.real, b.imag)
        kind = self._kl_kind_for_forward()
        yr, yi, kl = ops.CplxLinearLRTFn.apply(input.real, input.imag, w.real, w.imag, br, bi,
                                               self.log_sigma2, er, ei, seed, offset, kind)
        if kind is not None:
            self._kl_put(kl, (w.real, w.imag, self.log_sigma2))
        return cplx.Cplx(yr, yi)


class CplxLinearVD(CplxLinearGaussian, SparsityStats, BaseARD):
    _kl_kind = "cplx_vd"


class CplxLinearARD(CplxLinearVD):
    _kl_kind = "cplx_ard"


class CplxBilinearGaussian(_CplxGaussianMixin, CplxBilinear):

    def __init__(self, in1_features, in2_features, out_features, bias=True, conjugate=True):
        super().__init__(in1_features, in2_features, out_features, bias=bias, conjugate=conjugate)
        self._init_variational()

    def forward(self, input1, input2, eps=None):
        if not self.training:
            return super().forward(input1, input2)
        w, b = self.weight, self.bias
        if eps is not None:
            er, ei, seed, offset = eps.real, eps.imag, 0, 0
        else:
            er, ei, seed, offset = self._draw_noise((*input1.shape[:-1], self.out_features), input1)
        br, bi = (None, None) if b is None else (b.real, b.imag)
        yr, yi = ops.CplxBilinearFn.apply(input1.real, input1.imag, input2.real, input2.imag, w.real,
                                          w.imag, br, bi, bool(self.conjugate), self.log_sigma2, er, ei,
                                          seed, offset)
        return cplx.Cplx(yr, yi)


class CplxBilinearVD(CplxBilinearGaussian, SparsityStats, BaseARD):
    _kl_kind = "cplx_vd"


class CplxBilinearARD(CplxBilinearVD):
    _kl_kind = "cplx_ard"


class CplxConv2dGaussian(_CplxGaussianMixin, CplxConv2d):
    def __init__(self, in_channels, out_channels, kernel_size, stride=1, padding=0, dilation=1,
                 groups=1, bias=True, padding_mode="zeros"):
        super().__init__(in_channels, out_channels, kernel_size, stride=stride, padding=padding,
                         dilation=dilation, groups=groups, bias=bias, padding_mode=padding_mode)
        if self.padding_mode != "zeros":
            raise ValueError(f"Only `zeros` padding mode is supported. Got `{self.padding_mode}`.")
        self._init_variational()

    def forward(self, input, eps=None):
        if not self.training:
            return super().forward(input)
        from ... import conv
        return conv.cplx_conv2d_lrt(self, input, eps)


class CplxConv2dVD(CplxConv2dGaussian, SparsityStats, BaseARD):
    _kl_kind = "cplx_vd"


class CplxConv2dARD(CplxConv2dVD):
    _kl_kind = "cplx_ard"


class CplxConv1dGaussian(_CplxGaussianMixin, CplxConv1d):
    def __init__(self, in_channels, out_channels, kernel_size, stride=1, padding=0, dilation=1,
                 groups=1, bias=True, padding_mode="zeros"):
        super().__init__(in_channels, out_channels, kernel_size, stride=stride, padding=padding,
                         dilation=dilation, groups=groups, bias=bias, padding_mode=padding_mode)
        if self.padding_mode != "zeros":
            raise ValueError(f"Only `zeros` padding mode is supported. Got `{self.padding_mode}`.")
        self._init_variational()

    def forward(self, input, eps=None):
        if not self.training:
            return super().forward(input)
        from ... import conv
# ... 34 lines not shown
```

cplxmodule_amd/nn/relevance/noise.py:

```python
import math
import torch


class _NoiseState:
    def __init__(self):
        self.mode = "philox"
        self._seed = None
        self.counter = 0
        self._dev = {}

    @property
    def seed(self):
        base = torch.initial_seed() if self._seed is None else self._seed
        return (base + getattr(self, "_rank", 0) * 0x9E3779B97F4A7C15) & 0xFFFFFFFFFFFFFFFF

    def fold_rank(self, rank):
        self._rank = int(rank)
        self._dev = {}

    def manual_seed(self, seed):
        self._seed, self.counter = int(seed), 0
        self._dev = {}

    def set_mode(self, mode):
        if mode not in ("philox", "philox-device", "torch", "tape"):
            raise ValueError("noise mode must be 'philox', 'philox-device', 'torch' or 'tape'")
        self.mode = mode

    def set_tape(self, tensors):
        self._tape = list(tensors)
        self.mode = "tape"

    def pop_tape(self, shape, like, complex_):
        if not getattr(self, "_tape", None):
            raise RuntimeError("noise tape exhausted")
        t = self._tape.pop(0).to(device=like.device, dtype=like.dtype)
        want = ((2, *shape) if complex_ else tuple(shape))
        if tuple(t.shape) != tuple(want):
            raise RuntimeError(f"noise tape entry has shape {tuple(t.shape)}, the layer needs {tuple(want)}")
        return t / math.sqrt(2) if complex_ else t

    def next(self, device=None):
        if self.mode == "philox-device":
            from ... import ops
            return ops.philox_advance(self.device_state(device)), 0
        self.counter += 1
        return self.seed & 0xFFFFFFFFFFFFFFFF, self.counter

    def device_state(self, device):
        device = torch.device(device)
        key = device.index if device.index is not None else torch.cuda.current_device()
        if key not in self._dev:
            seed = self.seed & 0xFFFFFFFFFFFFFFFF
            seed = seed - (1 << 64) if seed >= (1 << 63) else seed
            self._dev[key] = torch.tensor([seed, self.counter + 1], dtype=torch.int64,
                                          device=device)
        return self._dev[key]


noise = _NoiseState()
```

cplxmodule_amd/nn/relevance/real.py:

```python
import torch

from .base import BaseARD, KLFusion
from .noise import noise
from ..utils.sparsity import SparsityStats
from ... import ops


class _RealGaussianMixin(KLFusion):
    _kl_kind = "real_vd"
    __sparsity_ignore__ = ("log_sigma2",)

    def _init_variational(self):
        self.log_sigma2 = torch.nn.Parameter(torch.empty(*self.weight.shape))
        self.reset_variational_parameters()

    def reset_variational_parameters(self):
        self.log_sigma2.data.fill_(-10.0)

    @property
    def log_alpha(self):
        return ops.LogAlphaFn.apply(self.log_sigma2, self.weight, None)

    @property
    def penalty(self):
        return ops.PenaltyFn.apply(self._kl_kind, self.log_sigma2, self.weight, None)

    def _penalty_reduced(self, reduction):
        total = self._kl_get((self.weight, self.log_sigma2))
        if total is None:
            total = ops.PenaltySumFn.apply(self._kl_kind, self.log_sigma2, self.weight, None)
        return total / self.log_sigma2.numel() if reduction == "mean" else total

    def relevance(self, *, threshold, **kwargs):
        with torch.no_grad():
            return ops.relevance_mask(self.weight, None, self.log_sigma2, threshold)

    def sparsity(self, *, threshold, **kwargs):
        with torch.no_grad():
            _, kept = ops.relevance_mask(self.weight, None, self.log_sigma2, threshold, count=True)
        return [(id(self.weight), self.weight.numel() - float(kept.item()))]

    def _draw_noise(self, shape, like):
        if noise.mode == "torch":
            return torch.randn(*shape, dtype=like.dtype, device=like.device), 0, 0
        if noise.mode == "tape":
            return noise.pop_tape(shape, like, False), 0, 0
        seed, offset = noise.next(like.device)
        return None, seed, offset


class LinearGaussian(_RealGaussianMixin, torch.nn.Linear):
    def __init__(self, in_features, out_features, bias=True):
        super().__init__(in_features, out_features, bias=bias)
        self._init_variational()

    def forward(self, input, eps=None):
        if not self.training:
            return ops.RealLinearFn.apply(input, self.weight, self.bias)
        seed = offset = 0
        if eps is None:
            eps, seed, offset = self._draw_noise((*input.shape[:-1], self.out_features), input)
        kind = self._kl_kind_for_forward()
        y, kl = ops.RealLinearLRTFn.apply(input, self.weight, self.bias, self.log_sigma2, eps,
                                          seed, offset, kind)
        if kind is not None:
            self._kl_put(kl, (self.weight, self.log_sigma2))
        return y


class LinearVD(LinearGaussian, SparsityStats, BaseARD):
    _kl_kind = "real_vd"


class LinearARD(LinearVD):
    _kl_kind = "real_ard"


class BilinearGaussian(_RealGaussianMixin, torch.nn.Bilinear):

    def __init__(self, in1_features, in2_features, out_features, bias=True):
        super().__init__(in1_features, in2_features, out_features, bias=bias)
        self._init_variational()

    def forward(self, input1, input2, eps=None):
        if not self.training:
            return ops.RealBilinearFn.apply(input1, input2, self.weight, self.bias, None, None, 0, 0)
        seed = offset = 0
        if eps is None:
            eps, seed, offset = self._draw_noise((*input1.shape[:-1], self.out_features), input1)
        return ops.RealBilinearFn.apply(input1, input2, self.weight, self.bias, self.log_sigma2, eps,
                                        seed, offset)


class BilinearVD(BilinearGaussian, SparsityStats, BaseARD):
    _kl_kind = "real_vd"


class BilinearARD(BilinearVD):
    _kl_kind = "real_ard"


class Conv2dGaussian(_RealGaussianMixin, torch.nn.Conv2d):
    def __init__(self, in_channels, out_channels, kernel_size, stride=1, padding=0, dilation=1,
                 groups=1, bias=True, padding_mode="zeros"):
        super().__init__(in_channels, out_channels, kernel_size, stride=stride, padding=padding,
                         dilation=dilation, groups=groups, bias=bias, padding_mode=padding_mode)
        if self.padding_mode != "zeros":
            raise ValueError(f"Only `zeros` padding mode is supported. Got `{self.padding_mode}`.")
        self._init_variational()

    def forward(self, input, eps=None):
        from ... import conv
        return conv.real_conv2d_layer(self, input, eps)


class Conv2dVD(Conv2dGaussian, SparsityStats, BaseARD):
    _kl_kind = "real_vd"


class Conv2dARD(Conv2dVD):
    _kl_kind = "real_ard"


class Conv1dGaussian(_RealGaussianMixin, torch.nn.Conv1d):
    def __init__(self, in_channels, out_channels, kernel_size, stride=1, padding=0, dilation=1,
                 groups=1, bias=True, padding_mode="zeros"):
        super().__init__(in_channels, out_channels, kernel_size, stride=stride, padding=padding,
                         dilation=dilation, groups=groups, bias=bias, padding_mode=padding_mode)
        if self.padding_mode != "zeros":
            raise ValueError(f"Only `zeros` padding mode is supported. Got `{self.padding_mode}`.")
        self._init_variational()

    def forward(self, input, eps=None):
        from ... import conv
        return conv.real_conv1d_layer(self, input, eps)


class Conv1dVD(Conv1dGaussian, SparsityStats, BaseARD):
    _kl_kind = "real_vd"


class Conv1dARD(Conv1dVD):
    _kl_kind = "real_ard"

# ... 22 lines not shown
```

cplxmodule_amd/ops.py:

```python
import ctypes
import os

import functools

import torch

from . import _lib, x3
from ._lib import CplxAmdError, call, dtype_code, launch_flags, ptr, require_device, scratch_key, stream_ptr, try_call

_ws_cache = {}


def once_differentiable(fn):
    @functools.wraps(fn)
    def wrapper(ctx, *args):
        with torch.no_grad():
            outputs = fn(ctx, *args)
        if not torch.is_grad_enabled():
            return outputs
        single = not isinstance(outputs, tuple)
        outs = (outputs,) if single else outputs
        live = [i for i, v in enumerate(outs) if isinstance(v, torch.Tensor) and v.is_floating_point()]
        if not live:
            return outputs
        err = torch._C._functions.DelayedError(
            b"trying to differentiate twice a function that was marked with @once_differentiable (cplxmodule_amd: this "
            b"backward is computed by raw HIP kernels; second derivatives exist for the linear layers, Cplx products and "
            b"matmul only)", len(live))
        wrapped = err(*[outs[i].detach().requires_grad_(True) for i in live])
        wrapped = (wrapped,) if isinstance(wrapped, torch.Tensor) else wrapped
        res = list(outs)
        for i, w in zip(live, wrapped):
            res[i] = w
        return res[0] if single else tuple(res)
    return wrapper


def _ws(device):
    key = scratch_key(device)
    if key not in _ws_cache:
        nbytes = int(_lib.load().cplxamd_vd_kl_ws_bytes())
        _ws_cache[key] = torch.empty(nbytes, dtype=torch.uint8, device=device)
    return _ws_cache[key]


def _c(t):
    return None if t is None else t.contiguous()


def _layout_of(t):
    if t.dim() == 4 and t.is_contiguous(memory_format=torch.channels_last) and not t.is_contiguous():
        return torch.channels_last
    return torch.contiguous_format


def _cf(t, fmt):
    return None if t is None else t.contiguous(memory_format=fmt)


def _f32(t):
    if t is not None and t.dtype != torch.float32:
        raise _lib.CplxAmdError(f"expected a float32 tensor, got {t.dtype}")
    return t


def cast(t, dtype):
    if t.dtype == dtype:
        return t
    require_device(t)
    t = _cf(t, _layout_of(t))
    out = torch.empty_like(t, dtype=dtype)
    call("cplxamd_cast", ptr(t), ptr(out), t.numel(), dtype_code(t), dtype_code(out), stream_ptr())
    return out


def transpose2d(t):
    require_device(t)
    t = t.contiguous()
    R, C = t.shape
    out = torch.empty(C, R, dtype=t.dtype, device=t.device)
    call("cplxamd_transpose", ptr(t), C, ptr(out), R, R, C, dtype_code(t), stream_ptr())
    return out


def colsum(t, out=None):
    require_device(t)
    t = t.contiguous()
    R, C = t.shape
    if out is None or not (out.is_contiguous() and out.dtype == torch.float32 and out.numel() == C):
        dst, out = out, torch.empty(C, dtype=torch.float32, device=t.device)
    else:
        dst = None
    ws = torch.empty(int(_lib.load().cplxamd_colsum_ws_bytes(C)), dtype=torch.uint8, device=t.device)
    call("cplxamd_colsum", ptr(t), C, ptr(out), R, C, dtype_code(t), ptr(ws), stream_ptr())
    return out if dst is None else dst.copy_(out)


def attach_colsum(t, sums):
    t._cplxamd_colsum = (sums, t.data_ptr(), t._version, tuple(t.shape))


def colsum_hint(t):
    h = getattr(t, "_cplxamd_colsum", None)
    if h is not None and h[1] == t.data_ptr() and h[2] == t._version and h[3] == tuple(t.shape) and h[0].numel() == t.shape[1]:
        return h[0]
    return None


def attach_scale(tr, ti, scale):
    tr._cplxamd_scale = (scale, tr.data_ptr(), tr._version, ti.data_ptr(), ti._version, tuple(tr.shape))


def scale_hint(tr, ti):
    h = getattr(tr, "_cplxamd_scale", None)
    if (h is not None and h[1] == tr.data_ptr() and h[2] == tr._version and h[3] == ti.data_ptr() and h[4] == ti._version
            and h[5] == tuple(tr.shape) == tuple(ti.shape)):
        return h[0]
    return None


def attach_wgrad(tr, ti, dw):
    tr._cplxamd_wgrad = (dw, tr.data_ptr(), tr._version, ti.data_ptr(), ti._version, tuple(tr.shape))


def wgrad_hint(tr, ti, node):
    h = getattr(tr, "_cplxamd_wgrad", None)
# ... 105 lines not shown

def cgemm(ar, ai, a_strides, br, bi, b_strides, M, N, K, bias=None, conj_b=False,
          out_dtype=torch.float32, out=None, accumulate=False, algo=0, beta=None, emul=None, scales=None):
    require_device(ar, ai, br, bi, emul)
    if out is None:
        cr = torch.empty(M, N, dtype=out_dtype, device=ar.device)
        ci = torch.empty(M, N, dtype=out_dtype, device=ar.device)
    else:
        cr, ci = out
    b_r, b_i = (None, None) if bias is None else bias
    ws = _gauss_ws(M, N, K, ar.device) if algo == 1 else _gemm_ws(M, N, K, True, ar, cr)
    beta = _beta(beta) if accumulate else None
    if ar.dtype == torch.float16:
        sa, sb = scales if scales is not None else (None, None)
        call("cplxamd_cgemm_sc_fl", ptr(ar), ptr(ai), a_strides[0], a_strides[1], ptr(br), ptr(bi), b_strides[0], b_strides[1],
             ptr(b_r), ptr(b_i), ptr(emul), ptr(cr), ptr(ci), N, M, N, K, int(conj_b), _lib.F16, int(accumulate), ptr(beta),
             ptr(sa), ptr(sb), ptr(ws), 0 if ws is None else ws.numel(), launch_flags(), stream_ptr())
        return cr, ci
    call("cplxamd_cgemm_fl", ptr(ar), ptr(ai), a_strides[0], a_strides[1], ptr(br), ptr(bi),
         b_strides[0], b_strides[1], ptr(b_r), ptr(b_i), ptr(emul), ptr(cr), ptr(ci), N, M, N, K,
         int(conj_b), dtype_code(ar), dtype_code(cr), int(accumulate), ptr(beta), int(algo), ptr(ws),
         0 if ws is None else ws.numel(), launch_flags(), stream_ptr())
    return cr, ci


def cgemm_batched(ar, ai, a_strides, br, bi, b_strides, batch, M, N, K, conj_b=False, out_dtype=None):
    require_device(ar, ai, br, bi)
    odt = out_dtype or ar.dtype
    cr = torch.empty(batch, M, N, dtype=odt, device=ar.device)
    ci = torch.empty_like(cr)
    call("cplxamd_cgemm_batched", ptr(ar), ptr(ai), *a_strides, ptr(br), ptr(bi), *b_strides, ptr(cr),
         ptr(ci), N, M * N, batch, M, N, K, int(conj_b), dtype_code(ar), dtype_code(cr), stream_ptr())
    return cr, ci


def einsum_desc(plan):
    d = _lib.EinsumDesc()
    for g, modes in enumerate(plan.groups):
        if len(modes) > 8:
            raise CplxAmdError("einsum: more than 8 modes in a group")
        d.nmodes[g] = len(modes)
        for i, md in enumerate(modes):
            d.extent[g][i], d.stride_a[g][i], d.stride_b[g][i], d.stride_c[g][i] = md.extent, md.sa, md.sb, md.sc
    return d


def ceinsum(ar, ai, br, bi, plan):
    require_device(ar, ai, br, bi)
    cr = torch.empty(plan.out_shape, dtype=ar.dtype, device=ar.device)
    ci = torch.empty_like(cr)
    d = einsum_desc(plan)
    call("cplxamd_ceinsum", ptr(ar), ptr(ai), ptr(br), ptr(bi), ptr(cr), ptr(ci), ctypes.byref(d), int(plan.conj_a),
         int(plan.conj_b), dtype_code(ar), dtype_code(cr), stream_ptr())
    return cr, ci


def rgemm(a, a_strides, b, b_strides, M, N, K, bias=None, emul=None, out_dtype=torch.float32,
          out=None, emul_exp=False, accumulate=False, beta=None, scales=None):
    require_device(a, b, bias, emul)
    c = torch.empty(M, N, dtype=out_dtype, device=a.device) if out is None else out
    ws = _gemm_ws(M, N, K, False, a, c)
    beta = _beta(beta) if accumulate else None
    if a.dtype == torch.float16:
        sa, sb = scales if scales is not None else (None, None)
        call("cplxamd_rgemm_sc_fl", ptr(a), a_strides[0], a_strides[1], ptr(b), b_strides[0], b_strides[1], ptr(bias), ptr(emul),
             int(emul_exp), ptr(c), N, M, N, K, _lib.F16, int(accumulate), ptr(beta), ptr(sa), ptr(sb), ptr(ws),
             0 if ws is None else ws.numel(), launch_flags(), stream_ptr())
        return c
    call("cplxamd_rgemm_fl", ptr(a), a_strides[0], a_strides[1], ptr(b), b_strides[0], b_strides[1],
         ptr(bias), ptr(emul), int(emul_exp), ptr(c), N, M, N, K, dtype_code(a), dtype_code(c),
         int(accumulate), ptr(beta), ptr(ws), 0 if ws is None else ws.numel(), launch_flags(), stream_ptr())
    return c


def philox_normal(n, seed, offset, device, complex_=False):
    er = torch.empty(n, dtype=torch.float32, device=device)
    ei = torch.empty(n, dtype=torch.float32, device=device) if complex_ else None
    require_device(er)
    call("cplxamd_philox_normal", ptr(er), ptr(ei), seed, offset, n, stream_ptr())
    return (er, ei) if complex_ else er


def _noise_args(seed, offset):
    if isinstance(seed, torch.Tensor):
        return 0, 0, ptr(seed)
    return seed, offset, None


def philox_advance(state):
    used = torch.empty_like(state)
    call("cplxamd_philox_advance", ptr(state), ptr(used), stream_ptr())
    return used


def _al16(t):
    return t if t is None or t.data_ptr() % 16 == 0 else t.clone()


def _s2(s2, like):
    return s2 if (s2.dtype == torch.bfloat16 and like.dtype == torch.bfloat16) else _f32(s2)


def _s2_dtype(x):
    return torch.bfloat16 if x.dtype == torch.bfloat16 else torch.float32


def reparam_fwd(mu_r, mu_i, s2, eps=None, seed=0, offset=0, inplace=False):
    require_device(mu_r, mu_i, s2)
    fmt = _layout_of(mu_r)
    mu_r, mu_i, s2 = _al16(_cf(mu_r, fmt)), _al16(_cf(mu_i, fmt)), _al16(_s2(_cf(s2, fmt), mu_r))
    e_r = e_i = None
    if eps is not None:
        e_r, e_i = eps if isinstance(eps, (tuple, list)) else (eps, None)
        e_r, e_i = _cf(cast(e_r, mu_r.dtype), fmt), (None if e_i is None else _cf(cast(e_i, mu_r.dtype), fmt))
        e_r, e_i = _al16(e_r), _al16(e_i)
    y_r = mu_r if inplace else torch.empty_like(mu_r)
    y_i = None if mu_i is None else (mu_i if inplace else torch.empty_like(mu_i))
    sd, of, st = _noise_args(seed, offset)
    call("cplxamd_lrt_reparam_fwd_ex", ptr(mu_r), ptr(mu_i), ptr(s2), ptr(e_r), ptr(e_i), sd,
         of, st, ptr(y_r), ptr(y_i), mu_r.numel(), dtype_code(mu_r), dtype_code(s2), stream_ptr())
    return y_r, y_i


def _colsum_ws(device, nbytes):
    key = scratch_key(device)
    buf = _colsum_ws_cache.get(key)
    if buf is None or buf.numel() < nbytes:
        buf = _colsum_ws_cache[key] = torch.empty(max(nbytes, 1 << 20), dtype=torch.uint8, device=device)
    return buf


_colsum_ws_cache = {}


def _as_rows(t, rows, cols):
    if t.dim() == 4 and not t.is_contiguous():
        t = t.permute(0, 2, 3, 1)
    return t.reshape(rows, cols)


def reparam_bwd(g_r, g_i, s2, eps=None, seed=0, offset=0, out_dtype=torch.float32, bias_sums=None):
    require_device(g_r, g_i, s2)
    fmt = _layout_of(s2)
    g_r, g_i, s2 = _al16(_cf(g_r, fmt)), _al16(_cf(g_i, fmt)), _al16(_s2(_cf(s2, fmt), g_r))
    e_r = e_i = None
    if eps is not None:
        e_r, e_i = eps if isinstance(eps, (tuple, list)) else (eps, None)
        e_r, e_i = _cf(cast(e_r, g_r.dtype), fmt), (None if e_i is None else _cf(cast(e_i, g_r.dtype), fmt))
        e_r, e_i = _al16(e_r), _al16(e_i)
    g_s2 = torch.empty_like(s2, dtype=out_dtype)
    sd, of, st = _noise_args(seed, offset)
    if bias_sums is not None:
        rows, cols = int(bias_sums[0]), int(bias_sums[1])
        assert rows * cols == g_r.numel()
        outs = bias_sums[2] if len(bias_sums) > 2 and bias_sums[2] is not None else (None, None)
        ok = lambda t: t is not None and t.is_contiguous() and t.dtype == torch.float32 and t.numel() == cols
        sum_r = outs[0] if ok(outs[0]) else torch.empty(cols, dtype=torch.float32, device=g_r.device)
        sum_i = None if g_i is None else (outs[1] if ok(outs[1]) else torch.empty(cols, dtype=torch.float32, device=g_r.device))
        need = int(_lib.load().cplxamd_lrt_reparam_bwd_cols_ws_bytes(rows, cols))
        fused = need > 0
        if fused:
            ws = _colsum_ws(g_r.device, need)
            fused = try_call("cplxamd_lrt_reparam_bwd_cols", ptr(g_r), ptr(g_i), ptr(s2), ptr(e_r), ptr(e_i), sd, of, st,
                             ptr(g_s2), rows, cols, dtype_code(g_r), dtype_code(g_s2), dtype_code(s2), ptr(sum_r),
                             ptr(sum_i), ptr(ws), ws.numel(), stream_ptr())
        if not fused:
            call("cplxamd_lrt_reparam_bwd_ex", ptr(g_r), ptr(g_i), ptr(s2), ptr(e_r), ptr(e_i), sd, of, st,
                 ptr(g_s2), g_r.numel(), dtype_code(g_r), dtype_code(g_s2), dtype_code(s2), stream_ptr())
            if g_i is not None:
                a_r, a_i = _as_rows(g_r, rows, cols).contiguous(), _as_rows(g_i, rows, cols).contiguous()
                cws = torch.empty(int(_lib.load().cplxamd_colsum_ws_bytes(cols)), dtype=torch.uint8, device=g_r.device)
                call("cplxamd_colsum2", ptr(a_r), ptr(a_i), cols, ptr(sum_r), ptr(sum_i), rows, cols, dtype_code(a_r), ptr(cws),
                     stream_ptr())
            else:
                colsum(_as_rows(g_r, rows, cols), out=sum_r)
        for dst, src in zip(outs, (sum_r, sum_i)):
            if dst is not None and src is not None and dst is not src:
                dst.copy_(src.view_as(dst))
        return g_s2, (outs[0] if outs[0] is not None else sum_r), (None if g_i is None else (outs[1] if outs[1] is not None else sum_i))
    call("cplxamd_lrt_reparam_bwd_ex", ptr(g_r), ptr(g_i), ptr(s2), ptr(e_r), ptr(e_i), sd, of, st,
         ptr(g_s2), g_r.numel(), dtype_code(g_r), dtype_code(g_s2), dtype_code(s2), stream_ptr())
    return g_s2


def lrt_dx_accum(dxr, dxi, xr, xi, ga):
    require_device(dxr, dxi, xr, xi, ga)
    call("cplxamd_lrt_dx_accum", ptr(dxr), ptr(dxi), ptr(xr), ptr(xi), ptr(ga), dxr.numel(),
         dtype_code(dxr), dtype_code(ga), stream_ptr())


def kl_fwd(kind, wr, wi, ls2, elementwise=False, total=True):
    require_device(wr, wi, ls2)
    wr, wi, ls2 = _f32(_c(wr)), _f32(_c(wi)), _f32(_c(ls2))
    elem = torch.empty_like(wr) if elementwise else None
    tot = torch.empty((), dtype=torch.float32, device=wr.device) if total else None
    call("cplxamd_vd_kl_fwd", ptr(wr), ptr(wi), ptr(ls2), _lib.KL_KINDS[kind], ptr(elem), ptr(tot),
         ptr(_ws(wr.device)), wr.numel(), stream_ptr())
    return elem, tot


def kl_bwd(kind, wr, wi, ls2, g_elem=None, g_scalar=None, need=(True, True, True)):
    require_device(wr, wi, ls2, g_elem, g_scalar)
    wr, wi, ls2 = _f32(_c(wr)), _f32(_c(wi)), _f32(_c(ls2))
    g_elem = _f32(_c(g_elem))
    if g_scalar is not None:
        g_scalar = _f32(g_scalar.reshape(()).contiguous())
    g_ls2 = torch.empty_like(ls2) if need[0] else None
    g_wr = torch.empty_like(wr) if need[1] else None
    g_wi = torch.empty_like(wi) if (wi is not None and need[2]) else None
    call("cplxamd_vd_kl_bwd", ptr(wr), ptr(wi), ptr(ls2), _lib.KL_KINDS[kind], ptr(g_elem),
         ptr(g_scalar), ptr(g_ls2), ptr(g_wr), ptr(g_wi), wr.numel(), stream_ptr())
    return g_ls2, g_wr, g_wi


def kl_fwd_bwd(kind, wr, wi, ls2, gscale=1.0):
    require_device(wr, wi, ls2)
    wr, wi, ls2 = _f32(_c(wr)), _f32(_c(wi)), _f32(_c(ls2))
    tot = torch.empty((), dtype=torch.float32, device=wr.device)
    g_ls2, g_wr = torch.empty_like(ls2), torch.empty_like(wr)
    g_wi = None if wi is None else torch.empty_like(wi)
    call("cplxamd_vd_kl_fwd_bwd", ptr(wr), ptr(wi), ptr(ls2), _lib.KL_KINDS[kind], float(gscale),
         ptr(tot), ptr(g_ls2), ptr(g_wr), ptr(g_wi), ptr(_ws(wr.device)), wr.numel(), stream_ptr())
    return tot, g_ls2, g_wr, g_wi


def prep_kl(kind, wr, wi, ls2, with_kl, grads=None):
    require_device(wr, wi, ls2)
    bf = torch.bfloat16
    wb = torch.empty_like(wr, dtype=bf)
    wib = None if wi is None else torch.empty_like(wi, dtype=bf)
    sb = torch.empty_like(ls2, dtype=bf)
    tot = None
    if with_kl:
        tot = torch.empty((), dtype=torch.float32, device=wr.device)
        if grads is None:
            grads = (torch.empty_like(ls2), torch.empty_like(wr), None if wi is None else torch.empty_like(wi))
    g = grads if with_kl else (None, None, None)
    call("cplxamd_vd_prep_kl", ptr(wr), ptr(wi), ptr(ls2), _lib.KL_KINDS.get(kind, 0), int(bool(with_kl)),
         ptr(wb), ptr(wib), ptr(sb), ptr(tot), ptr(g[0]), ptr(g[1]), ptr(g[2]),
         ptr(_ws(wr.device)) if with_kl else None, wr.numel(), stream_ptr())
    return wb, wib, sb, tot, (grads if with_kl else None)


def _prep_ok(x, *params):
    return (x.dtype == torch.bfloat16 and params[0].numel() % 4 == 0 and
            all(p is None or (p.dtype == torch.float32 and p.is_contiguous() and p.data_ptr() % 16 == 0)
                for p in params))


def log_alpha_bwd(g, wr, wi):
    require_device(g, wr, wi)
    g, wr, wi = _f32(_c(g)), _f32(_c(wr)), _f32(_c(wi))
    g_wr = torch.empty_like(wr)
    g_wi = None if wi is None else torch.empty_like(wi)
    call("cplxamd_vd_log_alpha_bwd", ptr(g), ptr(wr), ptr(wi), ptr(g_wr), ptr(g_wi), wr.numel(), stream_ptr())
    return g_wr, g_wi


def log_alpha(wr, wi, ls2):
    require_device(wr, wi, ls2)
    wr, wi, ls2 = _f32(_c(wr)), _f32(_c(wi)), _f32(_c(ls2))
    out = torch.empty_like(ls2)
    call("cplxamd_vd_log_alpha", ptr(wr), ptr(wi), ptr(ls2), ptr(out), wr.numel(), stream_ptr())
    return out


def relevance_mask(wr, wi, ls2, threshold, count=False):
    require_device(wr, wi, ls2)
    wr, wi, ls2 = _f32(_c(wr)), _f32(_c(wi)), _f32(_c(ls2))
    mask = torch.empty_like(ls2)
    cnt = torch.empty((), dtype=torch.int64, device=wr.device) if count else None
    call("cplxamd_vd_mask", ptr(wr), ptr(wi), ptr(ls2), float(threshold), ptr(mask), ptr(cnt),
         ptr(_ws(wr.device)), wr.numel(), stream_ptr())
    return (mask, cnt) if count else mask


def _is_bf16(t):
    return t.dtype == torch.bfloat16


class _Pieces:

    def __init__(self, *planes, abs2=False, made=None):
        self.planes, self.abs2, self.v = planes, abs2, made

    def get(self, kind):
        if self.v is None or self.v[0].kind != kind:
            if self.abs2:
                self.v = (x3.split(self.planes[0], op=x3.OP_ABS2, t2=self.planes[1] if len(self.planes) > 1 else None,
                                   kind=kind),)
            else:
                self.v = x3.split_planes(self.planes, kind=kind)
        return self.v

    def saved(self):
        if self.v is None:
            return (None,) * (len(self.planes) if not self.abs2 else 1) + (None,)
        return tuple(p.t for p in self.v) + (self.v[0].scale,)

    @staticmethod
    def restored(kind, tensors, scale):
        if kind is None or tensors[0] is None:
            return None
        n = 3 if kind == "x3" else 2
        return tuple(x3.Pieces(t, kind, scale, n) for t in tensors)


_X3_SAVE = os.environ.get("CPLXAMD_X3_SAVE", "1") != "0"


def _cplx_linear_fwd(x2r, x2i, wr, wi, bias, algo=0, mode=None, xs=None):
    B, I = x2r.shape
    O = wr.shape[0]
    kind = x3.take(B, O, I, x2r, x2i, wr, wi, mode=mode) if x2r.dtype == torch.float32 else None
    if kind:
        Xs = (xs or _Pieces(x2r, x2i)).get(kind)
        Ws = x3.split_planes((wr, wi), x3.SPLIT_B, kind=kind)
        yr, yi = x3.gemm_nn(Xs, Ws, B, O, I, bias=bias)
        return yr, yi, (wr, wi)
    wcr, wci = cast(wr, x2r.dtype), cast(wi, x2r.dtype)
    yr, yi = cgemm(x2r, x2i, (I, 1), wcr, wci, (I, 1), B, O, I, bias=bias, out_dtype=x2r.dtype,
# ... 181 lines not shown
        xs = _Pieces(x2r, x2i)
        yr, yi, ctx.wc = _cplx_linear_fwd(x2r, x2i, wmr, wmi, bias, algo, mode=ctx.mode, xs=xs)
        ctx.kind = x3.take(O, I, x2r.shape[0], mode=ctx.mode) if xs.v is not None else None
        keep = xs.saved() if (_X3_SAVE and ctx.kind and xs.v[0].kind == ctx.kind) else (None, None, None)
        ctx.save_for_backward(x2r, x2i, wr, wi, mask, *keep, xr, xi)
        ctx.has_bias = br is not None
        ctx.lead = xr.shape[:-1]
        return yr.view(*ctx.lead, O), yi.view(*ctx.lead, O)

    @staticmethod
    def backward(ctx, gr, gi):
        x2r, x2i, wr, wi, mask, xsr, xsi, xsc, xr0, xi0 = ctx.saved_tensors
        O, I = wr.shape
        need = ctx.needs_input_grad
        dxr = dxi = dwr = dwi = dbr = dbi = None
        if torch.is_grad_enabled():
            lin = lambda ar, ai, br, bi: CplxLinearFn.apply(ar, ai, br, bi, None, None, 0, None)
            G = (gr.reshape(-1, O), gi.reshape(-1, O))
            wmr, wmi = (wr, wi) if mask is None else (wr * mask, wi * mask)
            if need[0] or need[1]:
                dxr, dxi = lin(G[0], G[1], wmr.t(), -wmi.t())
                dxr, dxi = dxr.reshape(*ctx.lead, I), dxi.reshape(*ctx.lead, I)
            if need[2] or need[3]:
                dwr, dwi = lin(G[0].t(), G[1].t(), xr0.reshape(-1, I).t(), -xi0.reshape(-1, I).t())
                if mask is not None:
                    dwr, dwi = dwr * mask, dwi * mask
                dwr, dwi = dwr.to(wr.dtype), dwi.to(wi.dtype)
            if ctx.has_bias and (need[4] or need[5]):
                dbr, dbi = G[0].float().sum(0), G[1].float().sum(0)
            return dxr, dxi, dwr, dwi, dbr, dbi, None, None
        g2r, g2i = gr.reshape(-1, O).contiguous(), gi.reshape(-1, O).contiguous()
        gs = _Pieces(g2r, g2i)
        xs = _Pieces(x2r, x2i, made=_Pieces.restored(ctx.kind, (xsr, xsi), xsc))
        if need[2] or need[3]:
            dwr, dwi = grad_buffer(wr), grad_buffer(wi)
            _cplx_linear_dw(g2r, g2i, x2r, x2i, out=(dwr, dwi), algo=ctx.algo, emul=mask, mode=ctx.mode, gs=gs, xs=xs)
            _announce(wr, wi)
        if ctx.has_bias and (need[4] or need[5]):
            dbr, dbi = colsum2(g2r, g2i)
        if need[0] or need[1]:
            dxr, dxi = _cplx_linear_dx(g2r, g2i, ctx.wc[0], ctx.wc[1], x2r.dtype, ctx.algo, mode=ctx.mode, gs=gs)
            dxr, dxi = dxr.view(*ctx.lead, I), dxi.view(*ctx.lead, I)
        return dxr, dxi, dwr, dwi, dbr, dbi, None, None


def _kl_recompute(ctx):
    if tuple(t._version for t in ctx.kl_params) != ctx.kl_versions:
        raise RuntimeError("a parameter of this layer was modified in place between its forward pass and a "
                           "backward pass that has to recompute the KL gradients (e.g. optimizer.step() "
                           "with a retained graph): the recomputation would use the NEW values")
    if len(ctx.kl_params) == 3:
        wr, wi, ls2 = ctx.kl_params
        return kl_fwd_bwd(ctx.kl_kind, wr, wi, ls2)[1:]
    w, ls2 = ctx.kl_params
    r = kl_fwd_bwd(ctx.kl_kind, w, None, ls2)
    return (r[1], r[2])


class CplxLinearLRTFn(torch.autograd.Function):

    @staticmethod
    def forward(ctx, xr, xi, wr, wi, br, bi, ls2, eps_r, eps_i, seed, offset, kl_kind=None):
        require_device(xr, xi, wr, wi, br, bi, ls2, eps_r, eps_i)
        ctx.set_materialize_grads(False)
        O, I = wr.shape
        x2r, x2i = xr.reshape(-1, I).contiguous(), xi.reshape(-1, I).contiguous()
        B = x2r.shape[0]
        bias = None if br is None else (_f32(_c(br)), _f32(_c(bi)))
        wrc, wic, ls2c = _c(wr), _c(wi), _c(ls2)
        kl = ctx.klg = None
        if kl_kind is not None:
            ctx.klg = (grad_buffer(ls2), grad_buffer(wr), grad_buffer(wi))
            ctx.klg_shared = hook_of(ls2) is not None
        ctx.mode = mode = x3.get_fp32_mode()
        use3 = x3.take(B, O, I, x2r, x2i, wrc, wic, ls2c, mode=mode) if x2r.dtype == torch.float32 else None
        if _prep_ok(x2r, wrc, wic, ls2c):
            wcr, wci, S, kl, _ = prep_kl(kl_kind, wrc, wic, ls2c, kl_kind is not None, ctx.klg)
        else:
            wcr, wci = cast(wrc, x2r.dtype), cast(wic, x2r.dtype)
            S = None if use3 else exp(ls2c, out_dtype=x2r.dtype)
            if kl_kind is not None:
                kl = torch.empty((), dtype=torch.float32, device=x2r.device)
                g = ctx.klg
                call("cplxamd_vd_kl_fwd_bwd", ptr(_f32(wrc)), ptr(_f32(wic)), ptr(_f32(ls2c)), _lib.KL_KINDS[kl_kind],
                     1.0, ptr(kl), ptr(g[0]), ptr(g[1]), ptr(g[2]), ptr(_ws(x2r.device)), O * I, stream_ptr())
        ctx.wc, ctx.S = (wcr, wci), S
        keep = (None,) * 5
        ctx.kind = None
        if use3:
            xs, xa = _Pieces(x2r, x2i), _Pieces(x2r, x2i, abs2=True)
            mur, mui, _ = _cplx_linear_fwd(x2r, x2i, wcr, wci, bias, mode=mode, xs=xs)
            a = None
            s2 = x3.gemm_nn(xa.get(use3), (x3.split(ls2c, x3.SPLIT_B, op=x3.OP_EXP, kind=use3),), B, O, I)
            ctx.kind = x3.take(O, I, B, mode=mode)
            if _X3_SAVE and ctx.kind == use3:
                keep = (*xs.saved(), *xa.saved())
        else:
            mur, mui = cgemm(x2r, x2i, (I, 1), wcr, wci, (I, 1), B, O, I, bias=bias, out_dtype=x2r.dtype)
            a = abs2(x2r, x2i)
            s2 = rgemm(a, (I, 1), S, (I, 1), B, O, I, out_dtype=_s2_dtype(x2r))
        eps = None
        if eps_r is not None:
            eps = (eps_r.reshape(B, O), eps_i.reshape(B, O))
        yr, yi = reparam_fwd(mur, mui, s2, eps, seed, offset, inplace=True)
        ctx.save_for_backward(x2r, x2i, wr, wi, ls2, s2, a, eps_r, eps_i, br, bi, *keep)
        ctx.has_bias = br is not None
        ctx.lead, ctx.seed, ctx.offset = xr.shape[:-1], seed, offset
        ctx.kl_kind = kl_kind
        ctx.kl_params = (wr, wi, ls2) if kl_kind is not None else None
        ctx.kl_versions = tuple(t._version for t in ctx.kl_params) if kl_kind is not None else None
        return yr.view(*ctx.lead, O), yi.view(*ctx.lead, O), kl

    @staticmethod
    @once_differentiable
    def backward(ctx, gr, gi, gkl=None):
        need = ctx.needs_input_grad
        dxr = dxi = dwr = dwi = dbr = dbi = dls2 = None
        if gr is None and gi is None:
            if gkl is not None and ctx.kl_kind is not None:
                if ctx.klg is None:
                    ctx.klg, ctx.klg_shared = _kl_recompute(ctx), False
                dls2, dwr, dwi = (_scaled(gkl, t) for t in ctx.klg)
                if ctx.klg_shared:
                    ctx.klg = None
            ctx.kl_only_ran = True
            return dxr, dxi, dwr, dwi, dbr, dbi, dls2, None, None, None, None, None
        x2r, x2i, wr, wi, ls2, s2, a, eps_r, eps_i, br, bi, xsr, xsi, xsc, xsa, xac = _saved(ctx)
        O, I = wr.shape
        B = x2r.shape[0]
        klg = None
        if gkl is not None and ctx.kl_kind is not None:
            klg = _kl_recompute(ctx) if ctx.klg is None else ctx.klg
        g2r = torch.zeros(B, O, dtype=x2r.dtype, device=x2r.device) if gr is None else gr.reshape(B, O).contiguous()
        g2i = torch.zeros(B, O, dtype=x2r.dtype, device=x2r.device) if gi is None else gi.reshape(B, O).contiguous()
        eps = None if eps_r is None else (eps_r.reshape(B, O), eps_i.reshape(B, O))
        dt = x2r.dtype
        want_w, want_b = need[2] or need[3], ctx.has_bias and (need[4] or need[5])
        if want_b:
            gs2, dbr, dbi = reparam_bwd(g2r, g2i, s2, eps, ctx.seed, ctx.offset, out_dtype=dt,
                                        bias_sums=(B, O, (grad_buffer(br), grad_buffer(bi))))
        else:
            gs2 = reparam_bwd(g2r, g2i, s2, eps, ctx.seed, ctx.offset, out_dtype=dt)
        ls2c = _c(ls2)
        fused = klg is not None and klg is ctx.klg
        own = (lambda p: torch.empty(p.shape, dtype=torch.float32, device=p.device)) if (ctx.klg is not None and not fused) \
            else grad_buffer
        m3 = ctx.mode
        gs, g2s, xa = _Pieces(g2r, g2i), _Pieces(gs2), None
        xs = _Pieces(x2r, x2i, made=_Pieces.restored(ctx.kind, (xsr, xsi), xsc))
        if a is None:
            if x3.take(O, I, B, gs2, mode=m3):
                xa = _Pieces(x2r, x2i, abs2=True, made=_Pieces.restored(ctx.kind, (xsa,), xac))
            else:
                a = abs2(x2r, x2i)
        if want_w:
            if fused:
                dwr, dwi = klg[1], klg[2]
                _cplx_linear_dw(g2r, g2i, x2r, x2i, out=(dwr, dwi), accumulate=True, beta=gkl, mode=m3, gs=gs, xs=xs)
            else:
                dwr, dwi = own(wr), own(wi)
                _cplx_linear_dw(g2r, g2i, x2r, x2i, out=(dwr, dwi), mode=m3, gs=gs, xs=xs)
                if klg is not None:
                    dwr.add_(klg[1] * gkl)
                    dwi.add_(klg[2] * gkl)
            if _EARLY_W:
                _announce(wr, wi)
        if need[6]:
            if fused:
                dls2 = klg[0]
                _real_linear_dw(gs2, a, emul=ls2c, emul_exp=True, out=dls2, accumulate=True, beta=gkl, mode=m3, gs=g2s, xs=xa)
            else:
                dls2 = own(ls2)
                _real_linear_dw(gs2, a, emul=ls2c, emul_exp=True, out=dls2, mode=m3, gs=g2s, xs=xa)
                if klg is not None:
                    dls2.add_(klg[0] * gkl)
        if fused or getattr(ctx, "klg_shared", False):
            ctx.klg = None
        if not _EARLY_W:
            _announce(wr if dwr is not None else None, wi if dwi is not None else None)
        _announce(ls2 if dls2 is not None else None, br if dbr is not None else None, bi if dbi is not None else None)
        if need[0] or need[1]:
            if ctx.S is None:
                ga = _real_linear_dx(gs2, ls2c, dt, mode=m3, gs=g2s, w_exp=True)
            else:
                ga = _real_linear_dx(gs2, ctx.S, dt)
            dxr, dxi = _cplx_lrt_dx(g2r, g2i, ctx.wc[0], ctx.wc[1], x2r, x2i, ga, mode=m3, gs=gs)
            dxr, dxi = dxr.view(*ctx.lead, I), dxi.view(*ctx.lead, I)
# ... 15 lines not shown
        ctx.mode = x3.get_fp32_mode()
        xs = _Pieces(x2)
        y, wm = _real_linear_fwd(x2, wm, _c(b), mode=ctx.mode, xs=xs)
        ctx.wm = wm
        ctx.kind = x3.take(O, I, x2.shape[0], mode=ctx.mode) if xs.v is not None else None
        keep = xs.saved() if (_X3_SAVE and ctx.kind and xs.v[0].kind == ctx.kind) else (None, None)
        ctx.save_for_backward(x2, w, mask, *keep, x)
        ctx.has_bias, ctx.lead = b is not None, x.shape[:-1]
        return y.view(*ctx.lead, O)

    @staticmethod
    def backward(ctx, g):
        x2, w, mask, xsv, xsc, x0 = ctx.saved_tensors
        O, I = w.shape
        need = ctx.needs_input_grad
        dx = dw = db = None
        if torch.is_grad_enabled():
            lin = lambda a, b: RealLinearFn.apply(a, b, None, None)
            G = g.reshape(-1, O)
            wm = w if mask is None else w * mask
            if need[0]:
                dx = lin(G, wm.t()).reshape(*ctx.lead, I)
            if need[1]:
                dw = lin(G.t(), x0.reshape(-1, I).t())
                dw = (dw if mask is None else dw * mask).to(w.dtype)
            if ctx.has_bias and need[2]:
                db = G.float().sum(0)
            return dx, dw, db, None
        g2 = g.reshape(-1, O).contiguous()
        gs = _Pieces(g2)
        if need[1]:
            dw = grad_buffer(w)
            _real_linear_dw(g2, x2, emul=mask, out=dw, mode=ctx.mode, gs=gs,
                            xs=None if xsv is None else _Pieces(x2, made=_Pieces.restored(ctx.kind, (xsv,), xsc)))
            _announce(w)
        if ctx.has_bias and need[2]:
            db = colsum(g2)
        if need[0]:
            dx = _real_linear_dx(g2, ctx.wm, x2.dtype, mode=ctx.mode, gs=gs).view(*ctx.lead, I)
        return dx, dw, db, None


class MaskMulFn(torch.autograd.Function):

    @staticmethod
    def forward(ctx, wr, wi, mask):
        mask = _f32(_c(mask.expand_as(wr)))
        ctx.save_for_backward(mask)
        ctx.cplx = wi is not None
        our, oui = mask_mul(wr, wi, mask)
        return (our, oui) if ctx.cplx else our

    @staticmethod
    @once_differentiable
    def backward(ctx, gr, gi=None):
        (mask,) = ctx.saved_tensors
        dr, di = mask_mul(gr, gi if ctx.cplx else None, mask)
        return dr, di, None


class RealLinearLRTFn(torch.autograd.Function):

    @staticmethod
    def forward(ctx, x, w, b, ls2, eps, seed, offset, kl_kind=None):
        require_device(x, w, b, ls2, eps)
        ctx.set_materialize_grads(False)
        O, I = w.shape
        x2 = x.reshape(-1, I).contiguous()
        B = x2.shape[0]
        wc_, ls2c = _c(w), _c(ls2)
        kl = ctx.klg = None
        if kl_kind is not None:
            ctx.klg = (grad_buffer(ls2), grad_buffer(w))
            ctx.klg_shared = hook_of(ls2) is not None
        ctx.mode = mode = x3.get_fp32_mode()
        use3 = x3.take(B, O, I, x2, wc_, ls2c, mode=mode) if x2.dtype == torch.float32 else None
        if _prep_ok(x2, wc_, ls2c):
            wb, _, S, kl, _ = prep_kl(kl_kind, wc_, None, ls2c, kl_kind is not None,
                                      None if ctx.klg is None else (*ctx.klg, None))
        else:
            wb, S = cast(wc_, x2.dtype), (None if use3 else exp(ls2c, out_dtype=x2.dtype))
            if kl_kind is not None:
                kl = torch.empty((), dtype=torch.float32, device=x2.device)
                call("cplxamd_vd_kl_fwd_bwd", ptr(_f32(wc_)), None, ptr(_f32(ls2c)), _lib.KL_KINDS[kl_kind], 1.0,
                     ptr(kl), ptr(ctx.klg[0]), ptr(ctx.klg[1]), None, ptr(_ws(x2.device)), O * I, stream_ptr())
        ctx.wb, ctx.S = wb, S
        keep = (None,) * 4
        ctx.kind = None
        if use3:
            xs, xa = _Pieces(x2), _Pieces(x2, abs2=True)
            mu, _ = _real_linear_fwd(x2, wb, _c(b), mode=mode, xs=xs)
            a = None
            s2 = x3.gemm_nn(xa.get(use3), (x3.split(ls2c, x3.SPLIT_B, op=x3.OP_EXP, kind=use3),), B, O, I)
            ctx.kind = x3.take(O, I, B, mode=mode)
            if _X3_SAVE and ctx.kind == use3:
                keep = (*xs.saved(), *xa.saved())
        else:
            mu = rgemm(x2, (I, 1), wb, (I, 1), B, O, I, bias=_c(b), out_dtype=x2.dtype)
            a = abs2(x2)
            s2 = rgemm(a, (I, 1), S, (I, 1), B, O, I, out_dtype=_s2_dtype(x2))
        e = None if eps is None else eps.reshape(B, O)
        y, _ = reparam_fwd(mu, None, s2, e, seed, offset, inplace=True)
        ctx.save_for_backward(x2, w, ls2, s2, a, eps, b, *keep)
        ctx.has_bias, ctx.lead, ctx.seed, ctx.offset = b is not None, x.shape[:-1], seed, offset
        ctx.kl_kind = kl_kind
        ctx.kl_params = (w, ls2) if kl_kind is not None else None
        ctx.kl_versions = tuple(t._version for t in ctx.kl_params) if kl_kind is not None else None
        return y.view(*ctx.lead, O), kl

    @staticmethod
    @once_differentiable
    def backward(ctx, g, gkl=None):
        need = ctx.needs_input_grad
        dx = dw = db = dls2 = None
        if g is None:
            if gkl is not None and ctx.kl_kind is not None:
                if ctx.klg is None:
                    ctx.klg, ctx.klg_shared = _kl_recompute(ctx), False
                dls2, dw = _scaled(gkl, ctx.klg[0]), _scaled(gkl, ctx.klg[1])
                if ctx.klg_shared:
                    ctx.klg = None
            ctx.kl_only_ran = True
            return dx, dw, db, dls2, None, None, None, None
        x2, w, ls2, s2, a, eps, b, xsv, xsc, xsa, xac = _saved(ctx)
        O, I = w.shape
        B = x2.shape[0]
        klg = None
        if gkl is not None and ctx.kl_kind is not None:
            klg = _kl_recompute(ctx) if ctx.klg is None else ctx.klg
        g2 = g.reshape(B, O).contiguous()
        dt = x2.dtype
        e = None if eps is None else eps.reshape(B, O)
        if ctx.has_bias and need[2]:
            gs2, db, _ = reparam_bwd(g2, None, s2, e, ctx.seed, ctx.offset, out_dtype=dt,
                                     bias_sums=(B, O, (grad_buffer(b), None)))
        else:
            gs2 = reparam_bwd(g2, None, s2, e, ctx.seed, ctx.offset, out_dtype=dt)
        ls2c = _c(ls2)
        fused = klg is not None and klg is ctx.klg
        own = (lambda p: torch.empty(p.shape, dtype=torch.float32, device=p.device)) if (ctx.klg is not None and not fused) \
            else grad_buffer
        m3 = ctx.mode
        gs, g2s, xa = _Pieces(g2), _Pieces(gs2), None
        xs = None if xsv is None else _Pieces(x2, made=_Pieces.restored(ctx.kind, (xsv,), xsc))
        if a is None:
            if x3.take(O, I, B, gs2, mode=m3):
                xa = _Pieces(x2, abs2=True, made=_Pieces.restored(ctx.kind, (xsa,), xac))
            else:
                a = abs2(x2)
        if need[1]:
            if fused:
                dw = klg[1]
                _real_linear_dw(g2, x2, out=dw, accumulate=True, beta=gkl, mode=m3, gs=gs, xs=xs)
            else:
                dw = own(w)
                _real_linear_dw(g2, x2, out=dw, mode=m3, gs=gs, xs=xs)
                if klg is not None:
                    dw.add_(klg[1] * gkl)
        if need[3]:
            if fused:
                dls2 = klg[0]
                _real_linear_dw(gs2, a, emul=ls2c, emul_exp=True, out=dls2, accumulate=True, beta=gkl, mode=m3, gs=g2s, xs=xa)
            else:
                dls2 = own(ls2)
                _real_linear_dw(gs2, a, emul=ls2c, emul_exp=True, out=dls2, mode=m3, gs=g2s, xs=xa)
                if klg is not None:
                    dls2.add_(klg[0] * gkl)
        if fused or getattr(ctx, "klg_shared", False):
            ctx.klg = None
        _announce(ls2 if dls2 is not None else None, w if dw is not None else None, b if db is not None else None)
        if need[0]:
            if ctx.S is None:
                ga = _real_linear_dx(gs2, ls2c, dt, mode=m3, gs=g2s, w_exp=True)
            else:
                ga = _real_linear_dx(gs2, ctx.S, dt)
            dx = _real_lrt_dx(g2, ctx.wb if _is_bf16(g2) else _c(w), x2, ga, mode=m3, gs=gs)
            dx = dx.view(*ctx.lead, I)
        return dx, dw, db, dls2, None, None, None, None


def bilinear_reduce_fwd(u, t, bias, B, O, I1, conj):
    (ur, ui), (tr, ti) = u, t
    require_device(ur, ui, tr, ti)
    yr = torch.empty(B, O, dtype=tr.dtype, device=tr.device)
    yi = None if ti is None else torch.empty_like(yr)
# ... 617 lines not shown
```

include/cplxamd.h:

```cpp
#ifndef CPLXAMD_H
#define CPLXAMD_H

#include <stdint.h>

#ifdef __cplusplus
extern "C" {
#endif

#define CPLXAMD_ABI_VERSION 25

enum { CPLXAMD_F32 = 0, CPLXAMD_BF16 = 1,
       CPLXAMD_F16 = 2 ,
       CPLXAMD_F64 = 3  };

enum {
  CPLXAMD_ALGO_4M = 0,
  CPLXAMD_ALGO_3M = 1
};

enum {
  CPLXAMD_KL_REAL_VD = 0,
  CPLXAMD_KL_REAL_ARD = 1,
  CPLXAMD_KL_CPLX_VD = 2,
  CPLXAMD_KL_CPLX_ARD = 3,
  CPLXAMD_KL_CPLX_VD_APPROX = 4,
  CPLXAMD_KL_CPLX_VD_SCALEFREE = 5,
  CPLXAMD_KL_CPLX_VD_BOGUS = 6,
  CPLXAMD_KL_REAL_L0 = 7,
  CPLXAMD_KL_REAL_L1 = 8
};

enum {
  CPLXAMD_OK = 0,
  CPLXAMD_EINVAL = -1,
  CPLXAMD_EALIGN = -2,
  CPLXAMD_ESHAPE = -3,
  CPLXAMD_EWS = -4
};

enum {
  CPLXAMD_LAUNCH_DEFAULT = 0,
  CPLXAMD_LAUNCH_SHARED = 1,
  CPLXAMD_LAUNCH_EXCLUSIVE = 2,
  CPLXAMD_LAUNCH_FAMILY_SET = 0x100,
  CPLXAMD_LAUNCH_FAMILY_SHIFT = 16
};
#define CPLXAMD_LAUNCH_FAMILY(mask) (CPLXAMD_LAUNCH_FAMILY_SET | (((mask) & 0xff) << CPLXAMD_LAUNCH_FAMILY_SHIFT))

int cplxamd_abi_version(void);


int64_t cplxamd_vd_kl_ws_bytes(void);

int cplxamd_vd_kl_fwd(const float* wr, const float* wi, const float* log_sigma2, int kind,
                      float* out_elem, float* out_sum, void* ws, int64_t n, void* stream);

int cplxamd_vd_kl_bwd(const float* wr, const float* wi, const float* log_sigma2, int kind,
                      const float* g_elem, const float* g_scalar, float* g_log_sigma2,
                      float* g_wr, float* g_wi, int64_t n, void* stream);

int cplxamd_vd_kl_fwd_bwd(const float* wr, const float* wi, const float* log_sigma2, int kind,
                          float gscale, float* out_sum, float* g_log_sigma2, float* g_wr,
                          float* g_wi, void* ws, int64_t n, void* stream);

int cplxamd_vd_prep_kl(const float* wr, const float* wi, const float* log_sigma2, int kind, int with_kl,
                       void* wr_bf16, void* wi_bf16, void* s_bf16, float* out_sum, float* g_log_sigma2,
                       float* g_wr, float* g_wi, void* ws, int64_t n, void* stream);

int cplxamd_vd_log_alpha(const float* wr, const float* wi, const float* log_sigma2, float* out,
                         int64_t n, void* stream);

int cplxamd_vd_log_alpha_bwd(const float* g, const float* wr, const float* wi, float* g_wr, float* g_wi,
                             int64_t n, void* stream);

int cplxamd_vd_mask(const float* wr, const float* wi, const float* log_sigma2, float threshold,
                    float* mask, int64_t* count, void* ws, int64_t n, void* stream);

int cplxamd_expi_fwd(const float* x, float* y, int64_t n, void* stream);
int cplxamd_expi_bwd(const float* g, const float* x, float* gx, int64_t n, void* stream);

int cplxamd_lrt_reparam_fwd(const void* mu_r, const void* mu_i, const float* s2,
                            const void* eps_r, const void* eps_i, uint64_t seed,
                            uint64_t offset, const uint64_t* state, void* y_r, void* y_i,
                            int64_t n, int dtype, void* stream);

int cplxamd_lrt_reparam_bwd(const void* g_r, const void* g_i, const float* s2,
                            const void* eps_r, const void* eps_i, uint64_t seed,
                            uint64_t offset, const uint64_t* state, void* g_s2, int64_t n,
                            int dtype, int gs2_dtype, void* stream);

int cplxamd_lrt_reparam_fwd_ex(const void* mu_r, const void* mu_i, const void* s2,
                               const void* eps_r, const void* eps_i, uint64_t seed,
                               uint64_t offset, const uint64_t* state, void* y_r, void* y_i,
                               int64_t n, int dtype, int s2_dtype, void* stream);
int cplxamd_lrt_reparam_bwd_ex(const void* g_r, const void* g_i, const void* s2,
                               const void* eps_r, const void* eps_i, uint64_t seed,
                               uint64_t offset, const uint64_t* state, void* g_s2, int64_t n,
                               int dtype, int gs2_dtype, int s2_dtype, void* stream);

int64_t cplxamd_lrt_reparam_bwd_cols_ws_bytes(int64_t rows, int cols);
int cplxamd_lrt_reparam_bwd_cols(const void* g_r, const void* g_i, const void* s2,
                                 const void* eps_r, const void* eps_i, uint64_t seed,
                                 uint64_t offset, const uint64_t* state, void* g_s2, int64_t rows,
                                 int cols, int dtype, int gs2_dtype, int s2_dtype, float* sum_r,
                                 float* sum_i, void* ws, int64_t ws_bytes, void* stream);

int cplxamd_philox_advance(uint64_t* state, uint64_t* used, void* stream);

int cplxamd_philox_normal(float* eps_r, float* eps_i, uint64_t seed, uint64_t offset,
                          int64_t n, void* stream);

enum { CPLXAMD_L0_COLS = 1, CPLXAMD_L0_TRAIN = 2, CPLXAMD_L0_HARD = 4 };
int cplxamd_l0_gate_fwd(const void* a, const float* log_alpha, const float* u, uint64_t seed, uint64_t offset,
                        const uint64_t* state, const float* bias, void* out, int64_t rows, int cols, int mode,
                        int a_dtype, int out_dtype, double* total, void* ws, void* stream);
int64_t cplxamd_l0_gate_bwd_ws_bytes(int64_t rows, int cols);
int cplxamd_l0_gate_bwd(const void* d, const void* a, const float* log_alpha, const float* u, uint64_t seed,
                        uint64_t offset, const uint64_t* state, void* da, void* az, float* d_log_alpha, int64_t rows,
                        int cols, int mode, int d_dtype, int a_dtype, int da_dtype, int az_dtype, void* ws,
                        int64_t ws_bytes, void* stream);
int cplxamd_l1_mask(const float* w, float threshold, uint8_t* mask, double* count, void* ws, int64_t n, void* stream);
int cplxamd_philox_uniform(float* u, uint64_t seed, uint64_t offset, int64_t n, void* stream);

int cplxamd_cgemm(const void* a_r, const void* a_i, int64_t a_rs, int64_t a_cs,
                  const void* b_r, const void* b_i, int64_t b_rs, int64_t b_cs,
                  const float* bias_r, const float* bias_i, void* c_r, void* c_i, int64_t ldc,
                  int M, int N, int K, int conj_b, int in_dtype, int out_dtype, int accumulate,
                  int algo, void* ws, int64_t ws_bytes, void* stream);

int cplxamd_cgemm_ex(const void* a_r, const void* a_i, int64_t a_rs, int64_t a_cs,
                     const void* b_r, const void* b_i, int64_t b_rs, int64_t b_cs,
                     const float* bias_r, const float* bias_i, const float* emul, void* c_r, void* c_i,
                     int64_t ldc, int M, int N, int K, int conj_b, int in_dtype, int out_dtype, int accumulate,
                     const float* beta, int algo, void* ws, int64_t ws_bytes, void* stream);

int cplxamd_cgemm_fl(const void* a_r, const void* a_i, int64_t a_rs, int64_t a_cs,
                     const void* b_r, const void* b_i, int64_t b_rs, int64_t b_cs,
                     const float* bias_r, const float* bias_i, const float* emul, void* c_r, void* c_i,
                     int64_t ldc, int M, int N, int K, int conj_b, int in_dtype, int out_dtype, int accumulate,
                     const float* beta, int algo, void* ws, int64_t ws_bytes, int flags, void* stream);

int64_t cplxamd_cgemm3m_ws_bytes(int M, int N, int K);

int cplxamd_gemm_set_persistent(int on);

int cplxamd_gemm_set_family(int mask);

int64_t cplxamd_gemm_ws_bytes(int M, int N, int K, int cplx, int in_dtype, int out_dtype);

int cplxamd_cgemm_lrt_dx(const void* g_r, const void* g_i, int64_t g_rs, int64_t g_cs,
                         const void* w_r, const void* w_i, int64_t w_rs, int64_t w_cs,
                         const void* x_r, const void* x_i, const void* ga, int64_t ldx,
                         void* dx_r, void* dx_i, int64_t ldc, int M, int N, int K, int dtype, void* stream);
int cplxamd_rgemm_lrt_dx(const void* g, int64_t g_rs, int64_t g_cs, const void* w, int64_t w_rs, int64_t w_cs,
                         const void* x, const void* ga, int64_t ldx, void* dx, int64_t ldc, int M, int N, int K, int dtype,
                         void* stream);

int cplxamd_cgemm_lrt_dx_fl(const void* g_r, const void* g_i, int64_t g_rs, int64_t g_cs,
                            const void* w_r, const void* w_i, int64_t w_rs, int64_t w_cs,
                            const void* x_r, const void* x_i, const void* ga, int64_t ldx,
                            void* dx_r, void* dx_i, int64_t ldc, int M, int N, int K, int dtype, int flags, void* stream);
int cplxamd_rgemm_lrt_dx_fl(const void* g, int64_t g_rs, int64_t g_cs, const void* w, int64_t w_rs, int64_t w_cs,
                            const void* x, const void* ga, int64_t ldx, void* dx, int64_t ldc, int M, int N, int K,
                            int dtype, int flags, void* stream);
int cplxamd_rgemm_fl(const void* a, int64_t a_rs, int64_t a_cs, const void* b, int64_t b_rs,
                     int64_t b_cs, const float* bias, const float* emul, int emul_exp, void* c, int64_t ldc,
                     int M, int N, int K, int in_dtype, int out_dtype, int accumulate, const float* beta,
                     void* ws, int64_t ws_bytes, int flags, void* stream);
int cplxamd_gemm_plan(int cplx, int M, int N, int K, int ta, int tb, int out_dtype, int epi, int flags, int ncu);

int cplxamd_cgemm_batched(const void* a_r, const void* a_i, int64_t a_rs, int64_t a_cs, int64_t a_bs,
                          const void* b_r, const void* b_i, int64_t b_rs, int64_t b_cs, int64_t b_bs,
                          void* c_r, void* c_i, int64_t ldc, int64_t c_bs, int batch, int M, int N, int K,
                          int conj_b, int in_dtype, int out_dtype, void* stream);

int cplxamd_rgemm(const void* a, int64_t a_rs, int64_t a_cs, const void* b, int64_t b_rs,
                  int64_t b_cs, const float* bias, const float* emul, void* c, int64_t ldc,
                  int M, int N, int K, int in_dtype, int out_dtype, int accumulate, void* ws,
                  int64_t ws_bytes, void* stream);

int cplxamd_rgemm_ex(const void* a, int64_t a_rs, int64_t a_cs, const void* b, int64_t b_rs,
                     int64_t b_cs, const float* bias, const float* emul, int emul_exp, void* c, int64_t ldc,
                     int M, int N, int K, int in_dtype, int out_dtype, int accumulate, const float* beta,
                     void* ws, int64_t ws_bytes, void* stream);

int cplxamd_abs2(const void* xr, const void* xi, void* out, int64_t n, int in_dtype,
                 int out_dtype, void* stream);
int cplxamd_modulus(const float* xr, const float* xi, float* out, int64_t n, void* stream);
int cplxamd_cplx_abs_fwd(const void* xr, const void* xi, void* out, int64_t n, int dtype, void* stream);
int cplxamd_cplx_abs_bwd(const void* g, const void* xr, const void* xi, void* dxr, void* dxi, int64_t n,
// ... 299 lines not shown
```

Before: 2.518 million samples/s.

## Fold KL final reduction and Philox advance into producer kernels via tickets

Adds a sharded atomic ticket so the last-finishing block of the KL kernel performs the final sum, removing the separate kl_final launch. The reparam forward kernel also advances the Philox state in its last block, replacing a separate philox_advance launch. It changes the fused GEMM epilogue to load the shared gradient plane once per real/imag pair, and narrows the bwd column-reduction strip width. Risks are atomic and fence overhead, and correctness of the ticket reset under graph replay.

```diff
diff --git a/cplxmodule_amd/_lib.py b/cplxmodule_amd/_lib.py
--- a/cplxmodule_amd/_lib.py
+++ b/cplxmodule_amd/_lib.py
@@ -168,6 +168,8 @@
     "cplxamd_welch_fwd": [_P, _P, _L, _L, _L, _L, _P, _L, _L, _I, _D, _P, _P, _L, _I, _P],
     "cplxamd_welch_bwd": [_P, _P, _L, _L, _L, _L, _P, _L, _L, _I, _D, _P, _P, _P, _L, _L, _P, _L, _I, _P],
     "cplxamd_ceinsum": [_P, _P, _P, _P, _P, _P, _P, _I, _I, _I, _I, _P],
+    "cplxamd_ticket_ws_bytes": [],
+    "cplxamd_lrt_reparam_fwd_adv": [_P, _P, _P, _P, _P, _P, _P, _P, _L, _I, _I, _P],
 }
 
 
@@ -177,7 +179,8 @@
 
 
 CPLX_FN = {"exp": 0, "log": 1, "sin": 2, "cos": 3, "tan": 4, "sinh": 5, "cosh": 6, "tanh": 7}
-_RESTYPES = {"cplxamd_absmax_ws_bytes": c_int64, "cplxamd_conv2d_cl2_mom_chunks": c_int64, "cplxamd_conv2d_cl2_mom_chunks_fl": c_int64, "cplxamd_vd_kl_ws_bytes": c_int64, "cplxamd_lrt_reparam_bwd_cols_ws_bytes": c_int64, "cplxamd_l0_gate_bwd_ws_bytes": c_int64, "cplxamd_bn_ws_bytes": c_int64,
+KL_FOLD = 0x100
+_RESTYPES = {"cplxamd_ticket_ws_bytes": c_int64, "cplxamd_absmax_ws_bytes": c_int64, "cplxamd_conv2d_cl2_mom_chunks": c_int64, "cplxamd_conv2d_cl2_mom_chunks_fl": c_int64, "cplxamd_vd_kl_ws_bytes": c_int64, "cplxamd_lrt_reparam_bwd_cols_ws_bytes": c_int64, "cplxamd_l0_gate_bwd_ws_bytes": c_int64, "cplxamd_bn_ws_bytes": c_int64,
              "cplxamd_conv2d_wgrad_ws_bytes": c_int64, "cplxamd_conv2d_bf16_wgrad_ws_bytes": c_int64, "cplxamd_colsum_ws_bytes": c_int64, "cplxamd_gemm_ws_bytes": c_int64,
              "cplxamd_cgemm3m_ws_bytes": c_int64,
              "cplxamd_conv2d_nhwc_wgrad_ws_bytes": c_int64,
diff --git a/cplxmodule_amd/csrc/common.h b/cplxmodule_amd/csrc/common.h
--- a/cplxmodule_amd/csrc/common.h
+++ b/cplxmodule_amd/csrc/common.h
@@ -157,6 +157,29 @@
   if (wid == 0) r = wave_sum(r);
   __syncthreads();
   return r;
+}
+
+constexpr int kTicketShards = 16;
+constexpr int kTicketStride = 64;
+constexpr int kTicketWords = (1 + kTicketShards) * kTicketStride;
+
+__device__ __forceinline__ bool ticket_last(uint32_t* tick, uint32_t nblocks, uint32_t bid) {
+  const uint32_t shard = bid % kTicketShards;
+  const uint32_t members = (nblocks - shard + kTicketShards - 1) / kTicketShards;
+  const uint32_t nshards = nblocks < (uint32_t)kTicketShards ? nblocks : (uint32_t)kTicketShards;
+  uint32_t* mine = tick + (1 + shard) * kTicketStride;
+  asm volatile("s_waitcnt vmcnt(0)" ::: "memory");
+  __builtin_amdgcn_fence(__ATOMIC_RELEASE, "agent");
+  asm volatile("s_waitcnt vmcnt(0)" ::: "memory");
+  if (__hip_atomic_fetch_add(mine, 1u, __ATOMIC_RELAXED, __HIP_MEMORY_SCOPE_AGENT) != members - 1) return false;
+  __hip_atomic_store(mine, 0u, __ATOMIC_RELAXED, __HIP_MEMORY_SCOPE_AGENT);
+  __builtin_amdgcn_fence(__ATOMIC_ACQ_REL, "agent");
+  asm volatile("s_waitcnt vmcnt(0)" ::: "memory");
+  if (__hip_atomic_fetch_add(tick, 1u, __ATOMIC_RELAXED, __HIP_MEMORY_SCOPE_AGENT) != nshards - 1) return false;
+  __hip_atomic_store(tick, 0u, __ATOMIC_RELAXED, __HIP_MEMORY_SCOPE_AGENT);
+  __builtin_amdgcn_fence(__ATOMIC_ACQUIRE, "agent");
+  asm volatile("s_waitcnt vmcnt(0)" ::: "memory");
+  return true;
 }
 
 __device__ __forceinline__ uint64_t uniform64(uint64_t v) {
diff --git a/cplxmodule_amd/csrc/gemm_bf16_w4.hip b/cplxmodule_amd/csrc/gemm_bf16_w4.hip
--- a/cplxmodule_amd/csrc/gemm_bf16_w4.hip
+++ b/cplxmodule_amd/csrc/gemm_bf16_w4.hip
@@ -556,14 +556,17 @@
       const __amdgpu_buffer_rsrc_t rout0 = tile_rsrc(out_r, g.ldc, 2), rout1 = tile_rsrc(CPLX ? out_i : out_r, g.ldc, 2);
       const __amdgpu_buffer_rsrc_t rx0 = tile_rsrc(fuse ? g.fx_r : g.c_r, fuse ? g.fld : g.ldc, 2);
       const __amdgpu_buffer_rsrc_t rx1 = tile_rsrc(fuse ? (CPLX ? g.fx_i : g.fx_r) : g.c_r, fuse ? g.fld : g.ldc, 2);
-      constexpr int NR = NPL * (JB / 2) * (IB / 2);
+      constexpr int NH = (JB / 2) * (IB / 2), NR = NPL * NH;
+      auto plane_of = [](int r) { return fuse ? r % NPL : r / NH; };
+      auto jh_of = [](int r) { return ((fuse ? r / NPL : r) / (IB / 2)) % (JB / 2); };
+      auto ih_of = [](int r) { return (fuse ? r / NPL : r) % (IB / 2); };
       u32x4 gv[2][fuse ? 8 : 1], xv[2][fuse ? 8 : 1];
       auto load_ops = [&](int r) __attribute__((always_inline)) {
-        const int pl = r / ((JB / 2) * (IB / 2)), jh = (r / (IB / 2)) % (JB / 2), ih = r % (IB / 2);
+        const int pl = plane_of(r), jh = jh_of(r), ih = ih_of(r);
 #pragma unroll
         for (int pass = 0; pass < 8; ++pass) {
           const uint32_t so = (uint32_t)(ih * 8 + pass) * p8f + (uint32_t)(jh * 128);
-          gv[r & 1][pass] = ldb128(rga, vo_f, so);
+          if (pl == 0) gv[(r / NPL) & 1][pass] = ldb128(rga, vo_f, so);
           xv[r & 1][pass] = ldb128(pl ? rx1 : rx0, vo_f, so);
         }
       };
@@ -571,7 +574,7 @@
       if constexpr (PERSIST) W4_VMCNT(0);
 #pragma unroll
       for (int r = 0; r < NR; ++r) {
-        const int pl = r / ((JB / 2) * (IB / 2)), jh = (r / (IB / 2)) % (JB / 2), ih = r % (IB / 2);
+        const int pl = plane_of(r), jh = jh_of(r), ih = ih_of(r);
         const __amdgpu_buffer_rsrc_t rout = pl ? rout1 : rout0;
         if constexpr (fuse && !W4_EPI_PIPE) { if (r > 0) load_ops(r); }
 #pragma unroll
@@ -605,7 +608,7 @@
             for (int e = 0; e < 4; ++e) {
               const float d0 = __uint_as_float(v[e] << 16), d1 = __uint_as_float(v[e] & 0xffff0000u);
               const float x0 = __uint_as_float(xv[r & 1][pass][e] << 16), x1 = __uint_as_float(xv[r & 1][pass][e] & 0xffff0000u);
-              const float g0 = __uint_as_float(gv[r & 1][pass][e] << 16), g1 = __uint_as_float(gv[r & 1][pass][e] & 0xffff0000u);
+              const float g0 = __uint_as_float(gv[(r / NPL) & 1][pass][e] << 16), g1 = __uint_as_float(gv[(r / NPL) & 1][pass][e] & 0xffff0000u);
               ow[e] = pack_bf16(fmaf(2.0f * x0, g0, d0), fmaf(2.0f * x1, g1, d1));
             }
             stb128(ow, rout, vo_c, so);
diff --git a/cplxmodule_amd/csrc/kl.hip b/cplxmodule_amd/csrc/kl.hip
--- a/cplxmodule_amd/csrc/kl.hip
+++ b/cplxmodule_amd/csrc/kl.hip
@@ -202,6 +202,8 @@
   bf16_t* wr_b = nullptr;
   bf16_t* wi_b = nullptr;
   bf16_t* s_b = nullptr;
+  uint32_t* ticket = nullptr;
+  float* out_sum = nullptr;
 };
 
 __device__ __forceinline__ void st4g(float* p, const f4& v) {
@@ -372,6 +374,16 @@
   if (VALUE && a.partial) {
     const double s = block_sum<double, kKlThreads>(acc, red);
     if (threadIdx.x == 0) a.partial[blockIdx.x] = s;
+    if (a.ticket) {
+      if (threadIdx.x == 0) red[0] = ticket_last(a.ticket, gridDim.x, blockIdx.x) ? 1.0 : 0.0;
+      __syncthreads();
+      if (red[0] == 0.0) return;
+      __syncthreads();
+      double t = 0.0;
+      for (int i = threadIdx.x; i < (int)gridDim.x; i += kKlThreads) t += a.partial[i];
+      const double tot = block_sum<double, kKlThreads>(t, red);
+      if (threadIdx.x == 0) *a.out_sum = (float)tot;
+    }
   }
 }
 
@@ -417,6 +429,20 @@
     default:
       return CPLXAMD_EINVAL;
   }
+  CPLXAMD_CHECK_LAUNCH();
+  return 0;
+}
+
+template <bool GRAD>
+static int launch_kl_total(int kind, KlArgs a, int grid, float* out_sum, void* ws, hipStream_t st) {
+  const bool two = (kind & CPLXAMD_KL_FOLD) == 0;
+  if (!two) {
+    a.ticket = reinterpret_cast<uint32_t*>(static_cast<double*>(ws) + kKlMaxBlocks);
+    a.out_sum = out_sum;
+  }
+  int rc = launch_kl<true, GRAD>(kind & ~CPLXAMD_KL_FOLD, a, grid, st);
+  if (rc || !two) return rc;
+  kl_final_kernel<<<1, kKlThreads, 0, st>>>((const double*)ws, grid, out_sum);
   CPLXAMD_CHECK_LAUNCH();
   return 0;
 }
@@ -437,6 +463,7 @@
 }
 
 static bool kl_args_ok(const float* wr, const float* wi, const float* ls2, int kind, int64_t n) {
+  kind &= ~CPLXAMD_KL_FOLD;
   if (!wr || !ls2 || n < 0 || kind < 0 || kind > CPLXAMD_KL_REAL_L1) return false;
   const bool cplx = kind >= CPLXAMD_KL_CPLX_VD && kind <= CPLXAMD_KL_CPLX_VD_BOGUS;
   return cplx ? wi != nullptr : true;
@@ -573,7 +600,9 @@
 
 int cplxamd_abi_version(void) { return CPLXAMD_ABI_VERSION; }
 
-int64_t cplxamd_vd_kl_ws_bytes(void) { return (int64_t)kKlMaxBlocks * sizeof(double); }
+int64_t cplxamd_vd_kl_ws_bytes(void) { return (int64_t)kKlMaxBlocks * sizeof(double) + cplxamd_ticket_ws_bytes(); }
+
+int64_t cplxamd_ticket_ws_bytes(void) { return (int64_t)kTicketWords * sizeof(uint32_t); }
 
 int cplxamd_vd_kl_fwd(const float* wr, const float* wi, const float* log_sigma2, int kind,
                       float* out_elem, float* out_sum, void* ws, int64_t n, void* stream) {
@@ -582,13 +611,8 @@
   const int grid = stream_grid(n >> 2, kKlThreads);
   KlArgs a{wr, wi, log_sigma2, nullptr, nullptr, 1.0f, out_elem,
            out_sum ? (double*)ws : nullptr, nullptr, nullptr, nullptr, n};
-  int rc = launch_kl<true, false>(kind, a, grid, st);
-  if (rc) return rc;
-  if (out_sum) {
-    kl_final_kernel<<<1, kKlThreads, 0, st>>>((const double*)ws, grid, out_sum);
-    CPLXAMD_CHECK_LAUNCH();
-  }
-  return 0;
+  if (!out_sum) return launch_kl<true, false>(kind & ~CPLXAMD_KL_FOLD, a, grid, st);
+  return launch_kl_total<false>(kind, a, grid, out_sum, ws, st);
 }
 
 int cplxamd_vd_kl_bwd(const float* wr, const float* wi, const float* log_sigma2, int kind,
@@ -598,7 +622,7 @@
   const int grid = stream_grid(n >> 2, kKlThreads);
   KlArgs a{wr, wi, log_sigma2, g_elem, g_scalar, 1.0f, nullptr, nullptr,
            g_log_sigma2, g_wr, g_wi, n};
-  return launch_kl<false, true>(kind, a, grid, (hipStream_t)stream);
+  return launch_kl<false, true>(kind & ~CPLXAMD_KL_FOLD, a, grid, (hipStream_t)stream);
 }
 
 int cplxamd_vd_kl_fwd_bwd(const float* wr, const float* wi, const float* log_sigma2, int kind,
@@ -609,11 +633,7 @@
   const int grid = stream_grid(n >> 2, kKlThreads);
   KlArgs a{wr, wi, log_sigma2, nullptr, nullptr, gscale, nullptr, (double*)ws,
            g_log_sigma2, g_wr, g_wi, n};
-  int rc = launch_kl<true, true>(kind, a, grid, st);
-  if (rc) return rc;
-  kl_final_kernel<<<1, kKlThreads, 0, st>>>((const double*)ws, grid, out_sum);
-  CPLXAMD_CHECK_LAUNCH();
-  return 0;
+  return launch_kl_total<true>(kind, a, grid, out_sum, ws, st);
 }
 
 int cplxamd_vd_prep_kl(const float* wr, const float* wi, const float* log_sigma2, int kind, int with_kl,
@@ -633,11 +653,7 @@
   KlArgs a{wr, wi, log_sigma2, nullptr, nullptr, 1.0f, nullptr, (double*)ws,
            g_log_sigma2, g_wr, g_wi, n};
   a.wr_b = (bf16_t*)wr_bf16; a.wi_b = (bf16_t*)wi_bf16; a.s_b = (bf16_t*)s_bf16;
-  int rc = launch_kl<true, true>(kind, a, grid, st);
-  if (rc) return rc;
-  kl_final_kernel<<<1, kKlThreads, 0, st>>>((const double*)ws, grid, out_sum);
-  CPLXAMD_CHECK_LAUNCH();
-  return 0;
+  return launch_kl_total<true>(kind, a, grid, out_sum, ws, st);
 }
 
 int cplxamd_vd_log_alpha(const float* wr, const float* wi, const float* log_sigma2, float* out,
diff --git a/cplxmodule_amd/csrc/reparam.hip b/cplxmodule_amd/csrc/reparam.hip
--- a/cplxmodule_amd/csrc/reparam.hip
+++ b/cplxmodule_amd/csrc/reparam.hip
@@ -24,6 +24,7 @@
 }
 
 constexpr float kRsqrt2 = 0.70710678118654752f;
+constexpr int kColsTx = 64;
 
 template <bool CPLX>
 __device__ __forceinline__ void noise_vec(int64_t i4, uint64_t seed, uint64_t offset, f4& er,
@@ -59,10 +60,11 @@
   return lrt_std(s2);
 }
 
-template <typename T, typename TS, bool CPLX, bool PHILOX>
+template <typename T, typename TS, bool CPLX, bool PHILOX, bool ADV = false>
 __global__ __launch_bounds__(kRpThreads) void reparam_fwd_kernel(
     const T* mu_r, const T* mu_i, const TS* s2, const T* eps_r, const T* eps_i, uint64_t seed,
-    uint64_t offset, const uint64_t* state, T* y_r, T* y_i, int64_t n) {
+    uint64_t offset, const uint64_t* state, T* y_r, T* y_i, int64_t n, uint64_t* used = nullptr,
+    uint32_t* ticket = nullptr) {
   if (PHILOX && state) { seed = uniform64(state[0]); offset = uniform64(state[1]); }
   const int64_t n8 = n >> 3;
   const int64_t stride = (int64_t)gridDim.x * kRpThreads;
@@ -101,6 +103,16 @@
       const float sd = lrt_std_t<T>(io<TS>::ld(s2 + e));
       io<T>::st(y_r + e, io<T>::ld(mu_r + e) + er * sd);
       if (CPLX) io<T>::st(y_i + e, io<T>::ld(mu_i + e) + ei * sd);
+    }
+  }
+  if constexpr (ADV) {
+    asm volatile("s_waitcnt vmcnt(0) lgkmcnt(0)" ::: "memory");
+    __syncthreads();
+    if (threadIdx.x == 0 && ticket_last(ticket, gridDim.x, blockIdx.x)) {
+      uint64_t* st = const_cast<uint64_t*>(state);
+      used[0] = seed;
+      used[1] = offset;
+      st[1] = offset + 1;
     }
   }
 }
@@ -166,9 +178,9 @@
   __shared__ float red[kRpThreads * 16];
   if (PHILOX && state) { seed = uniform64(state[0]); offset = uniform64(state[1]); }
   const int CG = cols >> 3;
-  const int TX = CG < kRpThreads ? CG : kRpThreads, TY = kRpThreads / TX;
+  const int TX = CG < kColsTx ? CG : kColsTx, TY = kRpThreads / TX;
   const int tx = (int)threadIdx.x % TX, ty = (int)threadIdx.x / TX;
-  const int col = (int)blockIdx.x * (kRpThreads * 8) + tx * 8;
+  const int col0 = (int)blockIdx.x * (TX * 8), col = col0 + tx * 8;
   const int64_t r0 = (int64_t)blockIdx.y * rows_per_chunk;
   const int64_t r1 = r0 + rows_per_chunk < rows ? r0 + rows_per_chunk : rows;
   constexpr int NP = CPLX ? 2 : 1;
@@ -202,24 +214,17 @@
     st8(g_s2 + 8 * i, o);
   }
   float* dst = partial + (int64_t)blockIdx.y * NP * cols;
-  if (TY == 1) {
-#pragma unroll
-    for (int p = 0; p < NP; ++p) {
-      st4(dst + (int64_t)p * cols + col, f4{{acc[p][0], acc[p][1], acc[p][2], acc[p][3]}});
-      st4(dst + (int64_t)p * cols + col + 4, f4{{acc[p][4], acc[p][5], acc[p][6], acc[p][7]}});
-    }
-    return;
-  }
 #pragma unroll
   for (int p = 0; p < NP; ++p)
 #pragma unroll
     for (int c = 0; c < 8; ++c) red[((ty * NP + p) * TX + tx) * 8 + c] = acc[p][c];
   __syncthreads();
-  for (int f = (int)threadIdx.x; f < NP * cols; f += kRpThreads) {
-    const int p = f / cols, c = f % cols;
+  const int sw = TX * 8;
+  for (int f = (int)threadIdx.x; f < NP * sw; f += kRpThreads) {
+    const int p = f / sw, c = f % sw;
     float t = 0.0f;
     for (int l = 0; l < TY; ++l) t += red[((l * NP + p) * TX) * 8 + c];
-    dst[(int64_t)p * cols + c] = t;
+    dst[(int64_t)p * cols + col0 + c] = t;
   }
 }
 
@@ -248,8 +253,8 @@
   const int cg = cols / 8;
   if (cg < kRpThreads ? (kRpThreads % cg != 0) : (cols % (kRpThreads * 8) != 0)) return false;
   if (rows * (int64_t)cols >= ((int64_t)1 << 40)) return false;
-  p.strips = cg < kRpThreads ? 1 : cols / (kRpThreads * 8);
-  const int ty = cg < kRpThreads ? kRpThreads / cg : 1;
+  p.strips = cg < kColsTx ? 1 : cols / (kColsTx * 8);
+  const int ty = cg < kColsTx ? kRpThreads / cg : kRpThreads / kColsTx;
   int64_t chunks = rows / (16 * (int64_t)ty);
   const int64_t cap = 2048 / p.strips > 0 ? 2048 / p.strips : 1;
   if (chunks > cap) chunks = cap;
@@ -291,6 +296,20 @@
     er[e] = a;
     if (CPLX) ei[e] = b;
   }
+}
+
+template <typename T, typename TS>
+static int launch_fwd_adv(const void* mu_r, const void* mu_i, const void* s2, uint64_t* state, uint64_t* used,
+                          uint32_t* ticket, void* y_r, void* y_i, int64_t n, hipStream_t st) {
+  const int grid = stream_grid(n >> 3, kRpThreads);
+#define RP_FWDA(C)                                                                                    \
+  reparam_fwd_kernel<T, TS, C, true, true><<<grid, kRpThreads, 0, st>>>(                              \
+      (const T*)mu_r, (const T*)mu_i, (const TS*)s2, nullptr, nullptr, 0, 0, state, (T*)y_r, (T*)y_i, n, used, ticket)
+  if (mu_i) RP_FWDA(true);
+  else RP_FWDA(false);
+#undef RP_FWDA
+  CPLXAMD_CHECK_LAUNCH();
+  return 0;
 }
 
 template <typename T, typename TS>
@@ -363,6 +382,23 @@
     return launch_fwd<bf16_t, float>(mu_r, mu_i, s2, eps_r, eps_i, seed, offset, state, y_r, y_i, n, st);
   if (dtype == CPLXAMD_BF16 && s2_dtype == CPLXAMD_BF16)
     return launch_fwd<bf16_t, bf16_t>(mu_r, mu_i, s2, eps_r, eps_i, seed, offset, state, y_r, y_i, n, st);
+  return CPLXAMD_EINVAL;
+}
+
+int cplxamd_lrt_reparam_fwd_adv(const void* mu_r, const void* mu_i, const void* s2, uint64_t* state,
+                                uint64_t* used, void* tickets, void* y_r, void* y_i, int64_t n, int dtype,
+                                int s2_dtype, void* stream) {
+  if (!mu_r || !s2 || !y_r || !state || !used || !tickets || n < 0) return CPLXAMD_EINVAL;
+  if (!al16(mu_r) || !al16(mu_i) || !al16(s2) || !al16(y_r) || !al16(y_i)) return CPLXAMD_EALIGN;
+  if ((mu_i == nullptr) != (y_i == nullptr)) return CPLXAMD_EINVAL;
+  hipStream_t st = (hipStream_t)stream;
+  uint32_t* tk = (uint32_t*)tickets;
+  if (dtype == CPLXAMD_F32 && s2_dtype == CPLXAMD_F32)
+    return launch_fwd_adv<float, float>(mu_r, mu_i, s2, state, used, tk, y_r, y_i, n, st);
+  if (dtype == CPLXAMD_BF16 && s2_dtype == CPLXAMD_F32)
+    return launch_fwd_adv<bf16_t, float>(mu_r, mu_i, s2, state, used, tk, y_r, y_i, n, st);
+  if (dtype == CPLXAMD_BF16 && s2_dtype == CPLXAMD_BF16)
+    return launch_fwd_adv<bf16_t, bf16_t>(mu_r, mu_i, s2, state, used, tk, y_r, y_i, n, st);
   return CPLXAMD_EINVAL;
 }
 
diff --git a/cplxmodule_amd/nn/relevance/complex.py b/cplxmodule_amd/nn/relevance/complex.py
--- a/cplxmodule_amd/nn/relevance/complex.py
+++ b/cplxmodule_amd/nn/relevance/complex.py
@@ -56,14 +56,14 @@
         n_dropped = float(w.real.numel()) - float(kept.item())
         return [(id(w.real), n_dropped), (id(w.imag), n_dropped)]
 
-    def _draw_noise(self, shape, like):
+    def _draw_noise(self, shape, like, fold=False):
         if noise.mode == "torch":
             e = cplx.randn(*shape, dtype=like.dtype, device=like.device)
             return e.real, e.imag, 0, 0
         if noise.mode == "tape":
             e = noise.pop_tape(shape, like, True)
             return e[0], e[1], 0, 0
-        seed, offset = noise.next(like.device)
+        seed, offset = noise.next(like.device, fold=fold)
         return None, None, seed, offset
 
 
@@ -79,7 +79,7 @@
         if eps is not None:
             er, ei, seed, offset = eps.real, eps.imag, 0, 0
         else:
-            er, ei, seed, offset = self._draw_noise((*input.shape[:-1], self.out_features), input)
+            er, ei, seed, offset = self._draw_noise((*input.shape[:-1], self.out_features), input, fold=True)
         br, bi = (None, None) if b is None else (b.real, b.imag)
         kind = self._kl_kind_for_forward()
         yr, yi, kl = ops.CplxLinearLRTFn.apply(input.real, input.imag, w.real, w.imag, br, bi,
diff --git a/cplxmodule_amd/nn/relevance/noise.py b/cplxmodule_amd/nn/relevance/noise.py
--- a/cplxmodule_amd/nn/relevance/noise.py
+++ b/cplxmodule_amd/nn/relevance/noise.py
@@ -40,9 +40,11 @@
             raise RuntimeError(f"noise tape entry has shape {tuple(t.shape)}, the layer needs {tuple(want)}")
         return t / math.sqrt(2) if complex_ else t
 
-    def next(self, device=None):
+    def next(self, device=None, fold=False):
         if self.mode == "philox-device":
             from ... import ops
+            if fold:
+                return ops.PhiloxFold(self.device_state(device)), 0
             return ops.philox_advance(self.device_state(device)), 0
         self.counter += 1
         return self.seed & 0xFFFFFFFFFFFFFFFF, self.counter
diff --git a/cplxmodule_amd/nn/relevance/real.py b/cplxmodule_amd/nn/relevance/real.py
--- a/cplxmodule_amd/nn/relevance/real.py
+++ b/cplxmodule_amd/nn/relevance/real.py
@@ -40,12 +40,12 @@
             _, kept = ops.relevance_mask(self.weight, None, self.log_sigma2, threshold, count=True)
         return [(id(self.weight), self.weight.numel() - float(kept.item()))]
 
-    def _draw_noise(self, shape, like):
+    def _draw_noise(self, shape, like, fold=False):
         if noise.mode == "torch":
             return torch.randn(*shape, dtype=like.dtype, device=like.device), 0, 0
         if noise.mode == "tape":
             return noise.pop_tape(shape, like, False), 0, 0
-        seed, offset = noise.next(like.device)
+        seed, offset = noise.next(like.device, fold=fold)
         return None, seed, offset
 
 
@@ -59,7 +59,7 @@
             return ops.RealLinearFn.apply(input, self.weight, self.bias)
         seed = offset = 0
         if eps is None:
-            eps, seed, offset = self._draw_noise((*input.shape[:-1], self.out_features), input)
+            eps, seed, offset = self._draw_noise((*input.shape[:-1], self.out_features), input, fold=True)
         kind = self._kl_kind_for_forward()
         y, kl = ops.RealLinearLRTFn.apply(input, self.weight, self.bias, self.log_sigma2, eps,
                                           seed, offset, kind)
diff --git a/cplxmodule_amd/ops.py b/cplxmodule_amd/ops.py
--- a/cplxmodule_amd/ops.py
+++ b/cplxmodule_amd/ops.py
@@ -40,8 +40,22 @@
     key = scratch_key(device)
     if key not in _ws_cache:
         nbytes = int(_lib.load().cplxamd_vd_kl_ws_bytes())
-        _ws_cache[key] = torch.empty(nbytes, dtype=torch.uint8, device=device)
+        _ws_cache[key] = torch.zeros(nbytes, dtype=torch.uint8, device=device)
     return _ws_cache[key]
+
+
+def _tickets(device):
+    key = scratch_key(device)
+    if key not in _ticket_cache:
+        _ticket_cache[key] = torch.zeros(int(_lib.load().cplxamd_ticket_ws_bytes()), dtype=torch.uint8, device=device)
+    return _ticket_cache[key]
+
+
+_ticket_cache = {}
+
+
+def _kl_kind(kind, two_launch=False):
+    return _lib.KL_KINDS[kind] | (0 if two_launch else _lib.KL_FOLD)
 
 
 def _c(t):
@@ -313,9 +327,18 @@
 
 
 def _noise_args(seed, offset):
+    if isinstance(seed, PhiloxFold):
+        seed = seed.used
     if isinstance(seed, torch.Tensor):
         return 0, 0, ptr(seed)
     return seed, offset, None
+
+
+class PhiloxFold:
+    __slots__ = ("state", "used")
+
+    def __init__(self, state):
+        self.state, self.used = state, torch.empty_like(state)
 
 
 def philox_advance(state):
@@ -347,6 +370,10 @@
         e_r, e_i = _al16(e_r), _al16(e_i)
     y_r = mu_r if inplace else torch.empty_like(mu_r)
     y_i = None if mu_i is None else (mu_i if inplace else torch.empty_like(mu_i))
+    if isinstance(seed, PhiloxFold) and eps is None:
+        call("cplxamd_lrt_reparam_fwd_adv", ptr(mu_r), ptr(mu_i), ptr(s2), ptr(seed.state), ptr(seed.used),
+             ptr(_tickets(mu_r.device)), ptr(y_r), ptr(y_i), mu_r.numel(), dtype_code(mu_r), dtype_code(s2), stream_ptr())
+        return y_r, y_i
     sd, of, st = _noise_args(seed, offset)
     call("cplxamd_lrt_reparam_fwd_ex", ptr(mu_r), ptr(mu_i), ptr(s2), ptr(e_r), ptr(e_i), sd,
          of, st, ptr(y_r), ptr(y_i), mu_r.numel(), dtype_code(mu_r), dtype_code(s2), stream_ptr())
@@ -420,12 +447,12 @@
          dtype_code(dxr), dtype_code(ga), stream_ptr())
 
 
-def kl_fwd(kind, wr, wi, ls2, elementwise=False, total=True):
+def kl_fwd(kind, wr, wi, ls2, elementwise=False, total=True, two_launch=False):
     require_device(wr, wi, ls2)
     wr, wi, ls2 = _f32(_c(wr)), _f32(_c(wi)), _f32(_c(ls2))
     elem = torch.empty_like(wr) if elementwise else None
     tot = torch.empty((), dtype=torch.float32, device=wr.device) if total else None
-    call("cplxamd_vd_kl_fwd", ptr(wr), ptr(wi), ptr(ls2), _lib.KL_KINDS[kind], ptr(elem), ptr(tot),
+    call("cplxamd_vd_kl_fwd", ptr(wr), ptr(wi), ptr(ls2), _kl_kind(kind, two_launch), ptr(elem), ptr(tot),
          ptr(_ws(wr.device)), wr.numel(), stream_ptr())
     return elem, tot
 
@@ -444,18 +471,18 @@
     return g_ls2, g_wr, g_wi
 
 
-def kl_fwd_bwd(kind, wr, wi, ls2, gscale=1.0):
+def kl_fwd_bwd(kind, wr, wi, ls2, gscale=1.0, two_launch=False):
     require_device(wr, wi, ls2)
     wr, wi, ls2 = _f32(_c(wr)), _f32(_c(wi)), _f32(_c(ls2))
     tot = torch.empty((), dtype=torch.float32, device=wr.device)
     g_ls2, g_wr = torch.empty_like(ls2), torch.empty_like(wr)
     g_wi = None if wi is None else torch.empty_like(wi)
-    call("cplxamd_vd_kl_fwd_bwd", ptr(wr), ptr(wi), ptr(ls2), _lib.KL_KINDS[kind], float(gscale),
+    call("cplxamd_vd_kl_fwd_bwd", ptr(wr), ptr(wi), ptr(ls2), _kl_kind(kind, two_launch), float(gscale),
          ptr(tot), ptr(g_ls2), ptr(g_wr), ptr(g_wi), ptr(_ws(wr.device)), wr.numel(), stream_ptr())
     return tot, g_ls2, g_wr, g_wi
 
 
-def prep_kl(kind, wr, wi, ls2, with_kl, grads=None):
+def prep_kl(kind, wr, wi, ls2, with_kl, grads=None, two_launch=False):
     require_device(wr, wi, ls2)
     bf = torch.bfloat16
     wb = torch.empty_like(wr, dtype=bf)
@@ -467,7 +494,7 @@
         if grads is None:
             grads = (torch.empty_like(ls2), torch.empty_like(wr), None if wi is None else torch.empty_like(wi))
     g = grads if with_kl else (None, None, None)
-    call("cplxamd_vd_prep_kl", ptr(wr), ptr(wi), ptr(ls2), _lib.KL_KINDS.get(kind, 0), int(bool(with_kl)),
+    call("cplxamd_vd_prep_kl", ptr(wr), ptr(wi), ptr(ls2), _kl_kind(kind, two_launch) if with_kl else 0, int(bool(with_kl)),
          ptr(wb), ptr(wib), ptr(sb), ptr(tot), ptr(g[0]), ptr(g[1]), ptr(g[2]),
          ptr(_ws(wr.device)) if with_kl else None, wr.numel(), stream_ptr())
     return wb, wib, sb, tot, (grads if with_kl else None)
@@ -815,7 +842,7 @@
             if kl_kind is not None:
                 kl = torch.empty((), dtype=torch.float32, device=x2r.device)
                 g = ctx.klg
-                call("cplxamd_vd_kl_fwd_bwd", ptr(_f32(wrc)), ptr(_f32(wic)), ptr(_f32(ls2c)), _lib.KL_KINDS[kl_kind],
+                call("cplxamd_vd_kl_fwd_bwd", ptr(_f32(wrc)), ptr(_f32(wic)), ptr(_f32(ls2c)), _kl_kind(kl_kind),
                      1.0, ptr(kl), ptr(g[0]), ptr(g[1]), ptr(g[2]), ptr(_ws(x2r.device)), O * I, stream_ptr())
         ctx.wc, ctx.S = (wcr, wci), S
         keep = (None,) * 5
@@ -836,6 +863,8 @@
         if eps_r is not None:
             eps = (eps_r.reshape(B, O), eps_i.reshape(B, O))
         yr, yi = reparam_fwd(mur, mui, s2, eps, seed, offset, inplace=True)
+        if isinstance(seed, PhiloxFold):
+            seed = seed.used
         ctx.save_for_backward(x2r, x2i, wr, wi, ls2, s2, a, eps_r, eps_i, br, bi, *keep)
         ctx.has_bias = br is not None
         ctx.lead, ctx.seed, ctx.offset = xr.shape[:-1], seed, offset
@@ -1017,7 +1046,7 @@
             wb, S = cast(wc_, x2.dtype), (None if use3 else exp(ls2c, out_dtype=x2.dtype))
             if kl_kind is not None:
                 kl = torch.empty((), dtype=torch.float32, device=x2.device)
-                call("cplxamd_vd_kl_fwd_bwd", ptr(_f32(wc_)), None, ptr(_f32(ls2c)), _lib.KL_KINDS[kl_kind], 1.0,
+                call("cplxamd_vd_kl_fwd_bwd", ptr(_f32(wc_)), None, ptr(_f32(ls2c)), _kl_kind(kl_kind), 1.0,
                      ptr(kl), ptr(ctx.klg[0]), ptr(ctx.klg[1]), None, ptr(_ws(x2.device)), O * I, stream_ptr())
         ctx.wb, ctx.S = wb, S
         keep = (None,) * 4
@@ -1036,6 +1065,8 @@
             s2 = rgemm(a, (I, 1), S, (I, 1), B, O, I, out_dtype=_s2_dtype(x2))
         e = None if eps is None else eps.reshape(B, O)
         y, _ = reparam_fwd(mu, None, s2, e, seed, offset, inplace=True)
+        if isinstance(seed, PhiloxFold):
+            seed = seed.used
         ctx.save_for_backward(x2, w, ls2, s2, a, eps, b, *keep)
         ctx.has_bias, ctx.lead, ctx.seed, ctx.offset = b is not None, x.shape[:-1], seed, offset
         ctx.kl_kind = kl_kind
diff --git a/include/cplxamd.h b/include/cplxamd.h
--- a/include/cplxamd.h
+++ b/include/cplxamd.h
@@ -29,6 +29,7 @@
   CPLXAMD_KL_REAL_L0 = 7,
   CPLXAMD_KL_REAL_L1 = 8
 };
+enum { CPLXAMD_KL_FOLD = 0x100 };
 
 enum {
   CPLXAMD_OK = 0,
@@ -52,6 +53,8 @@
 
 int64_t cplxamd_vd_kl_ws_bytes(void);
 
+int64_t cplxamd_ticket_ws_bytes(void);
+
 int cplxamd_vd_kl_fwd(const float* wr, const float* wi, const float* log_sigma2, int kind,
                       float* out_elem, float* out_sum, void* ws, int64_t n, void* stream);
 
@@ -106,6 +109,10 @@
                                  float* sum_i, void* ws, int64_t ws_bytes, void* stream);
 
 int cplxamd_philox_advance(uint64_t* state, uint64_t* used, void* stream);
+
+int cplxamd_lrt_reparam_fwd_adv(const void* mu_r, const void* mu_i, const void* s2, uint64_t* state,
+                                uint64_t* used, void* tickets, void* y_r, void* y_i, int64_t n, int dtype,
+                                int s2_dtype, void* stream);
 
 int cplxamd_philox_normal(float* eps_r, float* eps_i, uint64_t seed, uint64_t offset,
                           int64_t n, void* stream);
```

Measured after the change: 2.369 million samples/s. 5.9% lower.
